# leotimus/binary-recommendation

Hardware: AMD Instinct MI355X
Metric: (user,item) pairs/sec at batch 65536 dim 64 (higher is better)
Workload: dtype f32; 1 GPU; NeuMF-A full training step (trainers/NFC_plain.py graph: 4 embeddings, 128->100->50->10->1, BCE, Keras-Adam adam_dense), embed_dim=64, 1000000 users x 100000 items per GPU, batch 65536 per GPU, uniform ids; global_batch=65536, parallelism=single GPU, steps_per_graph_launch=4, optimizer=adam_dense (deferred replay)

## Files before the change

### binary-recommendation_amd/csrc/adam_math.h

```cpp
#pragma once
#include "common.h"
#include "rows.h"

namespace br {

struct AdamHp {
  float alpha, b1, omb1, b2, omb2, eps;
  const float* alpha_ptr;
};
__device__ __forceinline__ void adam_resolve(AdamHp& h) {
  if (h.alpha_ptr) h.alpha = *h.alpha_ptr;
}

__device__ __forceinline__ float adam_inv_denom(float v, float eps) {
  return __builtin_amdgcn_rcpf(__builtin_amdgcn_sqrtf(v) + eps);
}

__device__ __forceinline__ void adam_update1(float& th, float& m, float& v, float g, const AdamHp& h) {
  m = __builtin_fmaf(h.omb1, g, h.b1 * m);
  v = __builtin_fmaf(h.omb2, g * g, h.b2 * v);
  th = __builtin_fmaf(-(h.alpha * m), adam_inv_denom(v, h.eps), th);
}
__device__ __forceinline__ void adam_update(float4& th, float4& m, float4& v, float4 g, const AdamHp& h) {
  adam_update1(th.x, m.x, v.x, g.x, h); adam_update1(th.y, m.y, v.y, g.y, h);
  adam_update1(th.z, m.z, v.z, g.z, h); adam_update1(th.w, m.w, v.w, g.w, h);
}
__device__ __forceinline__ void adam_update(float2& th, float2& m, float2& v, float2 g, const AdamHp& h) {
  adam_update1(th.x, m.x, v.x, g.x, h); adam_update1(th.y, m.y, v.y, g.y, h);
}
__device__ __forceinline__ void adam_update(float& th, float& m, float& v, float g, const AdamHp& h) {
  adam_update1(th, m, v, g, h);
}

typedef float pk2 __attribute__((ext_vector_type(2)));
__device__ __forceinline__ void adam_decay_pk(pk2& th, pk2& m, pk2& v, float alpha, const AdamHp& h) {
  m = m * h.b1;
  v = v * h.b2;
  pk2 d = {__builtin_amdgcn_sqrtf(v.x), __builtin_amdgcn_sqrtf(v.y)};
  d = d + h.eps;
  const pk2 r = {__builtin_amdgcn_rcpf(d.x), __builtin_amdgcn_rcpf(d.y)};
  th = __builtin_elementwise_fma(-(m * alpha), r, th);
}
__device__ __forceinline__ void adam_decay(float& th, float& m, float& v, float alpha, const AdamHp& h) {
  m = m * h.b1;
  v = v * h.b2;
  th = __builtin_fmaf(-(m * alpha), adam_inv_denom(v, h.eps), th);
}
__device__ __forceinline__ void adam_decay(float2& th, float2& m, float2& v, float alpha, const AdamHp& h) {
  pk2 t = {th.x, th.y}, mm = {m.x, m.y}, vv = {v.x, v.y};
  adam_decay_pk(t, mm, vv, alpha, h);
  th = make_float2(t.x, t.y); m = make_float2(mm.x, mm.y); v = make_float2(vv.x, vv.y);
}
__device__ __forceinline__ void adam_decay(float4& th, float4& m, float4& v, float alpha, const AdamHp& h) {
  pk2 t0 = {th.x, th.y}, m0 = {m.x, m.y}, v0 = {v.x, v.y}, t1 = {th.z, th.w}, m1 = {m.z, m.w}, v1 = {v.z, v.w};
  adam_decay_pk(t0, m0, v0, alpha, h);
  adam_decay_pk(t1, m1, v1, alpha, h);
  th = make_float4(t0.x, t0.y, t1.x, t1.y); m = make_float4(m0.x, m0.y, m1.x, m1.y); v = make_float4(v0.x, v0.y, v1.x, v1.y);
}

__device__ __forceinline__ bool all_zero(float4 a) { return a.x == 0.f && a.y == 0.f && a.z == 0.f && a.w == 0.f; }
__device__ __forceinline__ bool all_zero(float2 a) { return a.x == 0.f && a.y == 0.f; }
__device__ __forceinline__ bool all_zero(float a) { return a == 0.f; }

struct CatchUp {
  const float* m;
  const float* v;
  const int32_t* last;
  const StepStateDev* ss;
  float b1, b2, eps;
};

template <typename V>
__device__ __forceinline__ void adam_replay(V& th, V& m, V& v, uint32_t from, uint32_t upto, const float* ring, const AdamHp& h) {
  if (all_zero(m) && all_zero(v)) return;
  for (uint32_t j = from + 1; j <= upto; ++j) adam_decay(th, m, v, ring[j & (BR_ALPHA_RING - 1)], h);
}

template <typename V>
__device__ __forceinline__ void adam_replay_uniform(V& th, V& m, V& v, uint32_t from, uint32_t upto, const StepStateDev* __restrict__ ss,
                                                    const AdamHp& h) {
  if (__builtin_amdgcn_ballot_w64(!(all_zero(m) && all_zero(v))) == 0) return;
  float a = ss->alpha_hist[(from + 1) & (BR_ALPHA_RING - 1)];
  for (uint32_t j = from + 1; j <= upto; ++j) {
    const float an = ss->alpha_hist[(j + 1) & (BR_ALPHA_RING - 1)];
    adam_decay(th, m, v, a, h);
    a = an;
  }
}

struct FastRp {
  float c, eps_c;
  uint32_t trunc;
};
__device__ __forceinline__ FastRp fast_rp(const StepStateDev* __restrict__ ss) { return FastRp{ss->sqrt_b2, ss->eps_c, ss->trunc}; }

__device__ __forceinline__ void fast_open(pk2 v, float eps, pk2& d, pk2& r) {
  d = (pk2){__builtin_amdgcn_sqrtf(v.x), __builtin_amdgcn_sqrtf(v.y)} + eps;
  r = (pk2){__builtin_amdgcn_rcpf(d.x), __builtin_amdgcn_rcpf(d.y)};
}
__device__ __forceinline__ void fast_open(float v, float eps, float& d, float& r) {
  d = __builtin_amdgcn_sqrtf(v) + eps;
  r = __builtin_amdgcn_rcpf(d);
}
__device__ __forceinline__ void fast_step(pk2& th, pk2& m, pk2& d, pk2& r, float alpha, float b1, const FastRp& f) {
  m = m * b1;
  d = __builtin_elementwise_fma(d, (pk2){f.c, f.c}, (pk2){f.eps_c, f.eps_c});
  r = r * __builtin_elementwise_fma(-d, r, (pk2){2.f, 2.f});
  th = __builtin_elementwise_fma(-(m * alpha), r, th);
}
__device__ __forceinline__ void fast_step(float& th, float& m, float& d, float& r, float alpha, float b1, const FastRp& f) {
  m = m * b1;
  d = __builtin_fmaf(d, f.c, f.eps_c);
  r = r * __builtin_fmaf(-d, r, 2.f);
  th = __builtin_fmaf(-(m * alpha), r, th);
}
template <typename V> struct FastSt;
template <> struct FastSt<float> {
  float th, m, d, r;
  __device__ __forceinline__ void open(float t, float mm, float v, float eps) { th = t; m = mm; fast_open(v, eps, d, r); }
  __device__ __forceinline__ void step(float a, float b1, const FastRp& f) { fast_step(th, m, d, r, a, b1, f); }
  __device__ __forceinline__ float theta() const { return th; }
};
template <> struct FastSt<float2> {
  pk2 th, m, d, r;
  __device__ __forceinline__ void open(float2 t, float2 mm, float2 v, float eps) { th = (pk2){t.x, t.y}; m = (pk2){mm.x, mm.y}; fast_open((pk2){v.x, v.y}, eps, d, r); }
  __device__ __forceinline__ void step(float a, float b1, const FastRp& f) { fast_step(th, m, d, r, a, b1, f); }
  __device__ __forceinline__ float2 theta() const { return make_float2(th.x, th.y); }
};
template <> struct FastSt<float4> {
  pk2 th0, m0, d0, r0, th1, m1, d1, r1;
  __device__ __forceinline__ void open(float4 t, float4 mm, float4 v, float eps) {
    th0 = (pk2){t.x, t.y}; m0 = (pk2){mm.x, mm.y}; fast_open((pk2){v.x, v.y}, eps, d0, r0);
    th1 = (pk2){t.z, t.w}; m1 = (pk2){mm.z, mm.w}; fast_open((pk2){v.z, v.w}, eps, d1, r1);
  }
  __device__ __forceinline__ void step(float a, float b1, const FastRp& f) { fast_step(th0, m0, d0, r0, a, b1, f); fast_step(th1, m1, d1, r1, a, b1, f); }
  __device__ __forceinline__ float4 theta() const { return make_float4(th0.x, th0.y, th1.x, th1.y); }
};
__device__ __forceinline__ uint32_t pow_index(uint32_t k) { return k < (uint32_t)BR_ALPHA_RING ? k : (uint32_t)BR_ALPHA_RING - 1u; }

template <typename V>
__device__ __forceinline__ void fast_moments(V& m, V& v, uint32_t lag, const StepStateDev* __restrict__ ss) {
  const uint32_t k = pow_index(lag);
  m = vmul(m, ss->pow1[k]);
  v = vmul(v, ss->pow2[k]);
}

template <typename V>
__device__ __forceinline__ void adam_replay_fast_uniform(V& th, const V& m, const V& v, uint32_t from, uint32_t upto, const StepStateDev* __restrict__ ss,
                                                         const AdamHp& h) {
  if (__builtin_amdgcn_ballot_w64(!(all_zero(m) && all_zero(v))) == 0) return;
  const FastRp f = fast_rp(ss);
  const uint32_t lag = upto - from;
  const uint32_t end = from + (lag < f.trunc ? lag : f.trunc);
  FastSt<V> st;
  st.open(th, m, v, h.eps);
  uint32_t j = from + 1;
  for (; j + 7 <= end; j += 8) {
    const float* __restrict__ rp = ss->alpha_hist + (j & (BR_ALPHA_RING - 1));
    float a8[8];
#pragma unroll
    for (int k = 0; k < 8; ++k) a8[k] = rp[k];
#pragma unroll
    for (int k = 0; k < 8; ++k) st.step(a8[k], h.b1, f);
  }
  for (; j <= end; ++j) st.step(ss->alpha_hist[j & (BR_ALPHA_RING - 1)], h.b1, f);
  th = st.theta();
}
template <typename V>
__device__ __forceinline__ void adam_replay_fast(V& th, const V& m, const V& v, uint32_t from, uint32_t upto, const float* ring, const FastRp& f,
                                                 const AdamHp& h) {
  if (all_zero(m) && all_zero(v)) return;
  const uint32_t lag = upto - from;
  const uint32_t end = from + (lag < f.trunc ? lag : f.trunc);
  FastSt<V> st;
  st.open(th, m, v, h.eps);
  for (uint32_t j = from + 1; j <= end; ++j) st.step(ring[j & (BR_ALPHA_RING - 1)], h.b1, f);
  th = st.theta();
}

template <bool MOMENTS, typename V>
__device__ __forceinline__ void adam_catch_up_uniform(V& th, V& m, V& v, uint32_t from, uint32_t upto, const StepStateDev* __restrict__ ss, const AdamHp& h) {
  if (ss->fast) {
    adam_replay_fast_uniform(th, m, v, from, upto, ss, h);
    if (MOMENTS) fast_moments(m, v, upto - from, ss);
  } else {
    adam_replay_uniform(th, m, v, from, upto, ss, h);
  }
}
template <bool MOMENTS, typename V>
__device__ __forceinline__ void adam_catch_up(V& th, V& m, V& v, uint32_t from, uint32_t upto, const float* ring, const StepStateDev* __restrict__ ss,
                                              const AdamHp& h) {
  if (ss->fast) {
    adam_replay_fast(th, m, v, from, upto, ring, fast_rp(ss), h);
    if (MOMENTS) fast_moments(m, v, upto - from, ss);
  } else {
    adam_replay(th, m, v, from, upto, ring, h);
  }
}

__device__ __forceinline__ void stage_alpha_ring(float* lds_ring, const StepStateDev* ss) {
  for (int k = threadIdx.x; k < BR_ALPHA_RING; k += blockDim.x) lds_ring[k] = ss->alpha_hist[k];
  __syncthreads();
}

static inline AdamHp make_hp(double alpha, double b1, double b2, double eps) {
  AdamHp h;
  h.alpha = (float)alpha;
  h.b1 = (float)b1;
  h.omb1 = (float)(1.0 - b1);
  h.b2 = (float)b2;
  h.omb2 = (float)(1.0 - b2);
  h.eps = (float)eps;
  const StepStateDev* ss = current_step_state();
  h.alpha_ptr = ss ? &ss->alpha_t : nullptr;
  return h;
}

}
```

### binary-recommendation_amd/csrc/gather.hip

```cpp
#include "common.h"
#include "rows.h"
#include "adam_math.h"
#include "lookup_wave.h"

namespace br {

struct GatherArgs {
  const float* tables[4];
  const void* ids[4];
  float* outs[4];
  int64_t rows[4];
};

template <typename IdT, int VEC, int NT>
__global__ __launch_bounds__(256) void gather_rows_kernel(GatherArgs a, int dim, int chunks,
                                                           int lpr_log2, int64_t batch, int* err) {
  using V = typename VecT<VEC>::type;
  const int lpr = 1 << lpr_log2;
  const int64_t tid = (int64_t)blockIdx.x * blockDim.x + threadIdx.x;
  const int64_t b = tid >> lpr_log2;
  const int lir = (int)(tid & (lpr - 1));
  if (b >= batch) return;
  int64_t id[NT];
  bool ok[NT];
#pragma unroll
  for (int t = 0; t < NT; ++t) {
    id[t] = load_id(reinterpret_cast<const IdT*>(a.ids[t]), b);
    ok[t] = (uint64_t)id[t] < (uint64_t)a.rows[t];
    if (!ok[t] && err && lir == 0) *err = 1;
  }
  for (int c = lir; c < chunks; c += lpr) {
    V v[NT];
#pragma unroll
    for (int t = 0; t < NT; ++t)
      v[t] = ok[t] ? vload<VEC>(a.tables[t] + id[t] * dim + c * VEC) : vzero<VEC>();
#pragma unroll
    for (int t = 0; t < NT; ++t) vstore<VEC>(a.outs[t] + b * dim + c * VEC, v[t]);
  }
}

struct GatherSegJob { const float* table; int64_t rows; const void* ids; float* out; int64_t seg_off; };
struct GatherSegJobs { GatherSegJob j[2]; };
template <typename IdT, int VEC>
__global__ __launch_bounds__(256) void gather_rows_seg_kernel(GatherSegJobs jobs, int dim, int chunks, int lpr_log2, int64_t n, int64_t seg_len, int64_t seg_stride,
                                                               int64_t ld_out, int* err) {
  const GatherSegJob& jb = jobs.j[blockIdx.y];
  const int lpr = 1 << lpr_log2;
  const int64_t tid = (int64_t)blockIdx.x * blockDim.x + threadIdx.x;
  const int64_t b = tid >> lpr_log2;
  const int lir = (int)(tid & (lpr - 1));
  if (b >= n) return;
  const int64_t p = seg_phys(b, seg_len, seg_stride, jb.seg_off);
  const int64_t id = load_id((const IdT*)jb.ids, p);
  const bool ok = (uint64_t)id < (uint64_t)jb.rows;
  if (!ok && err && lir == 0) *err = 1;
  for (int c = lir; c < chunks; c += lpr)
    vstore<VEC>(jb.out + p * ld_out + c * VEC, ok ? vload<VEC>(jb.table + id * dim + c * VEC) : vzero<VEC>());
}

template <int VEC>
__global__ __launch_bounds__(256) void row_dot_kernel(const float* __restrict__ A, const float* __restrict__ Bm,
                                                       float* __restrict__ out, int dim, int chunks,
                                                       int lpr_log2, int64_t batch) {
  const int lpr = 1 << lpr_log2;
  const int64_t tid = (int64_t)blockIdx.x * blockDim.x + threadIdx.x;
  int64_t b = tid >> lpr_log2;
  const int lir = (int)(tid & (lpr - 1));
  const bool live = b < batch;
  if (!live) b = batch - 1;
  float s = 0.f;
  for (int c = lir; c < chunks; c += lpr)
    s += vdot(vload<VEC>(A + b * dim + c * VEC), vload<VEC>(Bm + b * dim + c * VEC));
  s = rowgroup_sum(s, lpr);
  if (live && lir == 0) out[b] = s;
}

template <int VEC>
__global__ __launch_bounds__(256) void row_dot_bwd_kernel(const float* __restrict__ A, const float* __restrict__ Bm,
                                                           const float* __restrict__ dout, float* __restrict__ dA,
                                                           float* __restrict__ dB, int dim, int chunks,
                                                           int lpr_log2, int64_t batch) {
  const int lpr = 1 << lpr_log2;
  const int64_t tid = (int64_t)blockIdx.x * blockDim.x + threadIdx.x;
  const int64_t b = tid >> lpr_log2;
  const int lir = (int)(tid & (lpr - 1));
  if (b >= batch) return;
  const float g = dout[b];
  for (int c = lir; c < chunks; c += lpr) {
    auto va = vload<VEC>(A + b * dim + c * VEC);
    auto vb = vload<VEC>(Bm + b * dim + c * VEC);
    vstore<VEC>(dA + b * dim + c * VEC, vmul(vb, g));
    vstore<VEC>(dB + b * dim + c * VEC, vmul(va, g));
  }
}

template <typename IdT, int VEC>
__global__ __launch_bounds__(256) void neumf_embed_fwd_kernel(
    const float* __restrict__ user_mlp, const float* __restrict__ item_mlp,
    const float* __restrict__ user_mf, const float* __restrict__ item_mf, int64_t ldu, int64_t ldi,
    int64_t user_rows, int64_t item_rows, const IdT* __restrict__ users, const IdT* __restrict__ items,
    int dim, int chunks, int lpr_log2, int64_t batch, int item_first, float* __restrict__ x0,
    float* __restrict__ dot, int* err, float* __restrict__ stash_user, float* __restrict__ stash_item, int64_t ld_stash) {
  using V = typename VecT<VEC>::type;
  const int lpr = 1 << lpr_log2;
  const int64_t tid = (int64_t)blockIdx.x * blockDim.x + threadIdx.x;
  int64_t b = tid >> lpr_log2;
  const int lir = (int)(tid & (lpr - 1));
  const bool live = b < batch;
  if (!live) b = batch - 1;
  const int64_t u = load_id(users, b), i = load_id(items, b);
  const bool uok = (uint64_t)u < (uint64_t)user_rows, iok = (uint64_t)i < (uint64_t)item_rows;
  if ((!uok || !iok) && err && lir == 0) *err = 1;
  float* xrow = x0 + b * (2 * (int64_t)dim);
  const int uoff = item_first ? dim : 0, ioff = item_first ? 0 : dim;
  float s = 0.f;
  for (int c = lir; c < chunks; c += lpr) {
    V um = uok ? vload<VEC>(user_mlp + u * ldu + c * VEC) : vzero<VEC>();
    V im = iok ? vload<VEC>(item_mlp + i * ldi + c * VEC) : vzero<VEC>();
    V uf = uok ? vload<VEC>(user_mf + u * ldu + c * VEC) : vzero<VEC>();
    V vf = iok ? vload<VEC>(item_mf + i * ldi + c * VEC) : vzero<VEC>();
    if (live) {
      vstore<VEC>(xrow + uoff + c * VEC, um);
      vstore<VEC>(xrow + ioff + c * VEC, im);
      if (stash_user) {
        vstore<VEC>(stash_user + b * ld_stash + c * VEC, uf);
        vstore<VEC>(stash_item + b * ld_stash + c * VEC, vf);
      }
    }
    s += vdot(uf, vf);
  }
  s = rowgroup_sum(s, lpr);
  if (live && lir == 0) dot[b] = s;
}

template <typename IdT, int VEC>
__global__ __launch_bounds__(256) void neumf_embed_fwd_deferred_kernel(
    const float* __restrict__ user_tab, const float* __restrict__ user_m, const float* __restrict__ user_v,
    const int32_t* __restrict__ user_last, const float* __restrict__ item_tab, const float* __restrict__ item_m,
    const float* __restrict__ item_v, const int32_t* __restrict__ item_last, int64_t user_rows, int64_t item_rows,
    const IdT* __restrict__ users, const IdT* __restrict__ items, int dim, int chunks, int lpr_log2, int64_t batch,
    int item_first, const StepStateDev* __restrict__ ss, AdamHp h, float* __restrict__ x0, float* __restrict__ dot,
    float* __restrict__ stash_user, float* __restrict__ stash_item, int64_t ld_stash, int* err) {
  using V = typename VecT<VEC>::type;
  __shared__ float ring[BR_ALPHA_RING];
  stage_alpha_ring(ring, ss);
  const int lpr = 1 << lpr_log2;
  const int64_t tid = (int64_t)blockIdx.x * blockDim.x + threadIdx.x;
  int64_t b = tid >> lpr_log2;
  const int lir = (int)(tid & (lpr - 1));
  const bool live = b < batch;
  if (!live) b = batch - 1;
  int64_t u = load_id(users, b), i = load_id(items, b);
  const bool uok = (uint64_t)u < (uint64_t)user_rows, iok = (uint64_t)i < (uint64_t)item_rows;
  if ((!uok || !iok) && err && lir == 0) *err = 1;
  if (!uok) u = 0;
  if (!iok) i = 0;
  const uint32_t t = ss->step;
  const uint32_t lu = (uint32_t)user_last[u], li = (uint32_t)item_last[i];
  const int64_t ld = 2 * (int64_t)dim;
  float* xrow = x0 + b * ld;
  const int uoff = item_first ? dim : 0, ioff = item_first ? 0 : dim;
  float s = 0.f;
  for (int c = lir; c < chunks; c += lpr) {
    const int64_t uo = u * ld + c * VEC, io = i * ld + c * VEC;
    V um = vload<VEC>(user_tab + uo), uf = vload<VEC>(user_tab + uo + dim);
    V im = vload<VEC>(item_tab + io), vf = vload<VEC>(item_tab + io + dim);
    if (lu + 1 < t) {
      V m0 = vload<VEC>(user_m + uo), v0 = vload<VEC>(user_v + uo), m1 = vload<VEC>(user_m + uo + dim), v1 = vload<VEC>(user_v + uo + dim);
      adam_catch_up<false>(um, m0, v0, lu, t - 1, ring, ss, h);
      adam_catch_up<false>(uf, m1, v1, lu, t - 1, ring, ss, h);
    }
    if (li + 1 < t) {
      V m0 = vload<VEC>(item_m + io), v0 = vload<VEC>(item_v + io), m1 = vload<VEC>(item_m + io + dim), v1 = vload<VEC>(item_v + io + dim);
      adam_catch_up<false>(im, m0, v0, li, t - 1, ring, ss, h);
      adam_catch_up<false>(vf, m1, v1, li, t - 1, ring, ss, h);
    }
    if (!uok) { um = vzero<VEC>(); uf = vzero<VEC>(); }
    if (!iok) { im = vzero<VEC>(); vf = vzero<VEC>(); }
    if (live) {
      vstore<VEC>(xrow + uoff + c * VEC, um);
      vstore<VEC>(xrow + ioff + c * VEC, im);
      vstore<VEC>(stash_user + b * ld_stash + c * VEC, uf);
      vstore<VEC>(stash_item + b * ld_stash + c * VEC, vf);
    }
    s += vdot(uf, vf);
  }
  s = rowgroup_sum(s, lpr);
  if (live && lir == 0) dot[b] = s;
}

template <typename IdT, int VEC>
__global__ __launch_bounds__(256) void neumf_embed_fwd_deferred_wave_kernel(const LookupArgs a) {
  const int64_t b = (int64_t)blockIdx.x * 4 + __builtin_amdgcn_readfirstlane((int)(threadIdx.x >> 6));
  if (b >= a.batch) return;
  lookup_wave_pair<IdT, VEC>(a, b, (int)(threadIdx.x & 63));
}

template <typename IdT, int VEC>
__global__ __launch_bounds__(256) void gather_rows_deferred_kernel(
    const float* __restrict__ table, const float* __restrict__ M, const float* __restrict__ Vv, const int32_t* __restrict__ last,
    int64_t rows, int dim, int chunks, int lpr_log2, const IdT* __restrict__ ids, int64_t n, const StepStateDev* __restrict__ ss,
    AdamHp h, float* __restrict__ out, int64_t ld_out, int* err) {
  using V = typename VecT<VEC>::type;
  __shared__ float ring[BR_ALPHA_RING];
  stage_alpha_ring(ring, ss);
  const int lpr = 1 << lpr_log2;
  const int64_t tid = (int64_t)blockIdx.x * blockDim.x + threadIdx.x;
  const int64_t b = tid >> lpr_log2;
  const int lir = (int)(tid & (lpr - 1));
  if (b >= n) return;
  int64_t r = load_id(ids, b);
  const bool ok = (uint64_t)r < (uint64_t)rows;
  if (!ok) { if (err && lir == 0) *err = 1; r = 0; }
  const uint32_t t = ss->step, seen = (uint32_t)last[r];
  for (int c = lir; c < chunks; c += lpr) {
    const int64_t off = r * dim + c * VEC;
    V th = vload<VEC>(table + off);
    if (seen + 1 < t) {
      V m = vload<VEC>(M + off), v = vload<VEC>(Vv + off);
      adam_catch_up<false>(th, m, v, seen, t - 1, ring, ss, h);
    }
    vstore<VEC>(out + b * ld_out + c * VEC, ok ? th : vzero<VEC>());
  }
}

template <typename IdT, int VEC>
__global__ __launch_bounds__(256) void gather_rows_deferred_wave_kernel(
    const float* __restrict__ table, const float* __restrict__ M, const float* __restrict__ Vv, const int32_t* __restrict__ last,
    int64_t rows, const IdT* __restrict__ ids, int64_t n, const StepStateDev* __restrict__ ss, AdamHp h, float* __restrict__ out,
    int64_t ld_out, int* err) {
  using V = typename VecT<VEC>::type;
  constexpr int dim = 64 * VEC;
  const int64_t b = (int64_t)blockIdx.x * 4 + __builtin_amdgcn_readfirstlane((int)(threadIdx.x >> 6));
  if (b >= n) return;
  const int lane = (int)(threadIdx.x & 63);
  int64_t r = load_id(ids, b);
  const bool ok = (uint64_t)r < (uint64_t)rows;
  if (!ok) { if (err && lane == 0) *err = 1; r = 0; }
  const uint32_t t = ss->step, seen = (uint32_t)last[r];
  const int64_t off = r * dim + lane * VEC;
  V th = vload<VEC>(table + off);
  if (seen + 1 < t) {
    V m = vload<VEC>(M + off), v = vload<VEC>(Vv + off);
    adam_catch_up_uniform<false>(th, m, v, seen, t - 1, ss, h);
  }
  vstore<VEC>(out + b * ld_out + lane * VEC, ok ? th : vzero<VEC>());
}

template <typename IdT, int VEC>
__global__ __launch_bounds__(256) void gather_rows_deferred_wave_pair_kernel(GatherDefJobs jobs, const StepStateDev* __restrict__ ss, AdamHp h,
                                                                              int64_t ld_out, int* err) {
  const GatherDefJob& jb = jobs.j[blockIdx.y];
  const int64_t b = (int64_t)blockIdx.x * 4 + __builtin_amdgcn_readfirstlane((int)(threadIdx.x >> 6));
  if (b >= jb.n) return;
  gather_deferred_wave_row<IdT, VEC>(jobs, jb, b, (int)(threadIdx.x & 63), ss, h, ld_out, err);
}

template <int VEC>
__global__ __launch_bounds__(256) void mf_grad_inplace_kernel(float* su, float* si, int64_t ld, const float* __restrict__ ddot,
                                                               int64_t batch, int chunks) {
  using V = typename VecT<VEC>::type;
  const int64_t e = (int64_t)blockIdx.x * blockDim.x + threadIdx.x;
  if (e >= batch * chunks) return;
  const int64_t b = e / chunks;
  const int c = (int)(e - b * chunks);
  const float g = ddot[b];
  const V u = vload<VEC>(su + b * ld + c * VEC), i = vload<VEC>(si + b * ld + c * VEC);
  vstore<VEC>(su + b * ld + c * VEC, vmul(i, g));
  vstore<VEC>(si + b * ld + c * VEC, vmul(u, g));
}

template <typename IdT, int VEC>
__global__ __launch_bounds__(256) void neumf_embed_bwd_kernel(
    const float* __restrict__ user_mf, const float* __restrict__ item_mf, int64_t ldu, int64_t ldi,
    int64_t user_rows, int64_t item_rows, const IdT* __restrict__ users, const IdT* __restrict__ items,
    int dim, int chunks, int lpr_log2, int64_t batch, int item_first, const float* __restrict__ dx0,
    const float* __restrict__ ddot, float* __restrict__ g_user_mlp, float* __restrict__ g_item_mlp,
    float* __restrict__ g_user_mf, float* __restrict__ g_item_mf, int64_t ldg, int out_by_id) {
  using V = typename VecT<VEC>::type;
  const int lpr = 1 << lpr_log2;
  const int64_t tid = (int64_t)blockIdx.x * blockDim.x + threadIdx.x;
  const int64_t b = tid >> lpr_log2;
  const int lir = (int)(tid & (lpr - 1));
  if (b >= batch) return;
  const int64_t u = load_id(users, b), i = load_id(items, b);
  const bool uok = (uint64_t)u < (uint64_t)user_rows, iok = (uint64_t)i < (uint64_t)item_rows;
  const int64_t ou = out_by_id ? (uok ? u : -1) : b, oi = out_by_id ? (iok ? i : -1) : b;
  const float g = ddot[b];
  const int uoff = item_first ? dim : 0, ioff = item_first ? 0 : dim;
  for (int c = lir; c < chunks; c += lpr) {
    V uf = uok ? vload<VEC>(user_mf + u * ldu + c * VEC) : vzero<VEC>();
    V vf = iok ? vload<VEC>(item_mf + i * ldi + c * VEC) : vzero<VEC>();
    if (ou >= 0) vstore<VEC>(g_user_mf + ou * ldg + c * VEC, vmul(vf, g));
    if (oi >= 0) vstore<VEC>(g_item_mf + oi * ldg + c * VEC, vmul(uf, g));
    if (g_user_mlp) {
      const float* xr = dx0 + b * (2 * (int64_t)dim);
      if (ou >= 0) vstore<VEC>(g_user_mlp + ou * ldg + c * VEC, vload<VEC>(xr + uoff + c * VEC));
      if (oi >= 0) vstore<VEC>(g_item_mlp + oi * ldg + c * VEC, vload<VEC>(xr + ioff + c * VEC));
    }
  }
}

template <typename IdT, int VEC>
__global__ __launch_bounds__(256) void bpr_fwd_bwd_kernel(
    const float* __restrict__ user_table, const float* __restrict__ item_table, int64_t user_rows,
    int64_t item_rows, const IdT* __restrict__ users, const IdT* __restrict__ pos,
    const IdT* __restrict__ neg, int dim, int chunks, int lpr_log2, int64_t batch, float inv_batch,
    float* __restrict__ per_triplet, double* __restrict__ loss_sum, float* __restrict__ g_user,
    float* __restrict__ g_item, int* err) {
  using V = typename VecT<VEC>::type;
  const int lpr = 1 << lpr_log2;
  const int64_t tid = (int64_t)blockIdx.x * blockDim.x + threadIdx.x;
  int64_t b = tid >> lpr_log2;
  const int lir = (int)(tid & (lpr - 1));
  const bool live = b < batch;
  if (!live) b = batch - 1;
  const int64_t u = load_id(users, b), p = load_id(pos, b), n = load_id(neg, b);
  const bool uok = (uint64_t)u < (uint64_t)user_rows;
  const bool pok = (uint64_t)p < (uint64_t)item_rows, nok = (uint64_t)n < (uint64_t)item_rows;
  if (!(uok && pok && nok) && err && lir == 0) *err = 1;
  float sp = 0.f, sn = 0.f;
  const bool one_pass = chunks <= lpr;
  V eu = vzero<VEC>(), ep = vzero<VEC>(), en = vzero<VEC>();
  if (one_pass) {
    if (lir < chunks) {
      eu = uok ? vload<VEC>(user_table + u * dim + lir * VEC) : vzero<VEC>();
      ep = pok ? vload<VEC>(item_table + p * dim + lir * VEC) : vzero<VEC>();
      en = nok ? vload<VEC>(item_table + n * dim + lir * VEC) : vzero<VEC>();
    }
    sp = vdot(eu, ep);
    sn = vdot(eu, en);
  } else {
    for (int c = lir; c < chunks; c += lpr) {
      V a = uok ? vload<VEC>(user_table + u * dim + c * VEC) : vzero<VEC>();
      V bp = pok ? vload<VEC>(item_table + p * dim + c * VEC) : vzero<VEC>();
      V bn = nok ? vload<VEC>(item_table + n * dim + c * VEC) : vzero<VEC>();
      sp += vdot(a, bp);
      sn += vdot(a, bn);
    }
  }
  sp = rowgroup_sum(sp, lpr);
  sn = rowgroup_sum(sn, lpr);
  const float x = sp - sn;
  const float s = sigmoidf_acc(x);
  const float l = 1.f - s;
  const float dx = -s * (1.f - s) * inv_batch;
  if (live) {
    if (per_triplet && lir == 0) per_triplet[b] = l;
    float* gu = g_user + b * dim;
    float* gp = g_item + b * dim;
    float* gn = g_item + (batch + b) * dim;
    if (one_pass) {
      if (lir < chunks) {
        vstore<VEC>(gu + lir * VEC, vmul(vsub(ep, en), dx));
        vstore<VEC>(gp + lir * VEC, vmul(eu, dx));
        vstore<VEC>(gn + lir * VEC, vmul(eu, -dx));
      }
    } else {
      for (int c = lir; c < chunks; c += lpr) {
        V a = uok ? vload<VEC>(user_table + u * dim + c * VEC) : vzero<VEC>();
        V bp = pok ? vload<VEC>(item_table + p * dim + c * VEC) : vzero<VEC>();
        V bn = nok ? vload<VEC>(item_table + n * dim + c * VEC) : vzero<VEC>();
        vstore<VEC>(gu + c * VEC, vmul(vsub(bp, bn), dx));
        vstore<VEC>(gp + c * VEC, vmul(a, dx));
        vstore<VEC>(gn + c * VEC, vmul(a, -dx));
      }
    }
  }
  __shared__ double red[4];
  double contrib = (live && lir == 0) ? (double)l : 0.0;
  contrib = wave_sum_d(contrib);
  const int wave = threadIdx.x >> 6, lane = threadIdx.x & 63;
  if (lane == 0) red[wave] = contrib;
  __syncthreads();
  if (threadIdx.x == 0 && loss_sum) atomicAdd(loss_sum + (blockIdx.x & (BR_SUM_SLOTS - 1)), red[0] + red[1] + red[2] + red[3]);
}

}

using namespace br;

static inline unsigned grid_for_rows(int64_t batch, int lpr_log2) {
  const int64_t rows_per_block = 256 >> lpr_log2;
  return (unsigned)ceil_div(batch, rows_per_block);
}

extern "C" int brGatherRows(int n_tables, const float* const* tables, const int64_t* table_rows,
                            const void* const* ids, float* const* outs, int dim, int64_t batch,
                            int id_type, int* err_flag, brStream stream) {
  BR_CHECK_ARG(n_tables >= 1 && n_tables <= BR_MAX_TABLES, "brGatherRows: n_tables %d out of [1,%d]", n_tables, BR_MAX_TABLES);
  BR_CHECK_ARG(dim >= 1 && batch >= 0, "brGatherRows: bad dim/batch");
  BR_CHECK_ARG(id_type == BR_IDS_I32 || id_type == BR_IDS_I64, "brGatherRows: bad id_type %d", id_type);
  if (batch == 0) return BR_OK;
  for (int t = 0; t < n_tables; ++t)
    BR_CHECK_ARG(tables[t] && outs[t] && table_rows[t] > 0, "brGatherRows: null table/out %d", t);
  const RowGeom g = row_geom(dim);
  hipStream_t s = (hipStream_t)stream;
  const unsigned grid = grid_for_rows(batch, g.lpr_log2);
  for (int t0 = 0; t0 < n_tables; t0 += 4) {
    const int nt = (n_tables - t0) < 4 ? (n_tables - t0) : 4;
    GatherArgs a{};
    for (int t = 0; t < nt; ++t) {
      a.tables[t] = tables[t0 + t];
      a.ids[t] = ids ? ids[t0 + t] : nullptr;
      a.outs[t] = outs[t0 + t];
      a.rows[t] = table_rows[t0 + t];
    }
#define LAUNCH_G(NT) \
  BR_DISPATCH_ID(id_type, BR_DISPATCH_VEC(g.vec, (gather_rows_kernel<IdT, VEC, NT><<<grid, 256, 0, s>>>(a, dim, g.chunks, g.lpr_log2, batch, err_flag))))
    switch (nt) {
      case 1: LAUNCH_G(1); break;
      case 2: LAUNCH_G(2); break;
      case 3: LAUNCH_G(3); break;
      default: LAUNCH_G(4); break;
    }
#undef LAUNCH_G
    BR_CHECK_LAUNCH("brGatherRows");
  }
  return BR_OK;
}

extern "C" int brRowDot(const float* a, const float* b, float* out, int dim, int64_t batch, brStream stream) {
  BR_CHECK_ARG(a && b && out && dim >= 1 && batch >= 0, "brRowDot: bad args");
  if (batch == 0) return BR_OK;
  const RowGeom g = row_geom(dim);
  BR_DISPATCH_VEC(g.vec, (row_dot_kernel<VEC><<<grid_for_rows(batch, g.lpr_log2), 256, 0, (hipStream_t)stream>>>(
                             a, b, out, dim, g.chunks, g.lpr_log2, batch)));
  BR_CHECK_LAUNCH("brRowDot");
  return BR_OK;
}

extern "C" int brRowDotBackward(const float* a, const float* b, const float* dout, float* da, float* db,
                                int dim, int64_t batch, brStream stream) {
  BR_CHECK_ARG(a && b && dout && da && db && dim >= 1 && batch >= 0, "brRowDotBackward: bad args");
  if (batch == 0) return BR_OK;
  const RowGeom g = row_geom(dim);
  BR_DISPATCH_VEC(g.vec, (row_dot_bwd_kernel<VEC><<<grid_for_rows(batch, g.lpr_log2), 256, 0, (hipStream_t)stream>>>(
                             a, b, dout, da, db, dim, g.chunks, g.lpr_log2, batch)));
  BR_CHECK_LAUNCH("brRowDotBackward");
  return BR_OK;
}

extern "C" int brNeumfEmbedForward(const float* user_mlp, const float* item_mlp, const float* user_mf,
                                   const float* item_mf, int64_t ld_user, int64_t ld_item, int64_t user_rows,
                                   int64_t item_rows, const void* users, const void* items, int id_type, int dim,
                                   int64_t batch, int item_first, float* x0, float* dot, int* err_flag, brStream stream) {
  return brNeumfEmbedForwardStash(user_mlp, item_mlp, user_mf, item_mf, ld_user, ld_item, user_rows, item_rows, users, items, id_type, dim, batch, item_first, x0, dot,
                                  nullptr, nullptr, 0, err_flag, stream);
}

extern "C" int brNeumfEmbedForwardStash(const float* user_mlp, const float* item_mlp, const float* user_mf,
                                        const float* item_mf, int64_t ld_user, int64_t ld_item, int64_t user_rows,
                                        int64_t item_rows, const void* users, const void* items, int id_type, int dim,
                                        int64_t batch, int item_first, float* x0, float* dot, float* stash_user, float* stash_item, int64_t ld_stash,
                                        int* err_flag, brStream stream) {
  BR_CHECK_ARG(user_mlp && item_mlp && user_mf && item_mf && x0 && dot, "brNeumfEmbedForward: null pointer");
  BR_CHECK_ARG((stash_user == nullptr) == (stash_item == nullptr) && (!stash_user || ld_stash >= dim), "brNeumfEmbedForwardStash: both stashes (ld >= dim) or neither");
  BR_CHECK_ARG(dim >= 1 && batch >= 0 && user_rows > 0 && item_rows > 0, "brNeumfEmbedForward: bad sizes");
  BR_CHECK_ARG(ld_user >= dim && ld_item >= dim, "brNeumfEmbedForward: row strides < dim");
  BR_CHECK_ARG(id_type == BR_IDS_I32 || id_type == BR_IDS_I64, "brNeumfEmbedForward: bad id_type");
  if (batch == 0) return BR_OK;
  const RowGeom g = row_geom_ld(dim, vec_width({ld_user, ld_item, stash_user ? ld_stash : 0}, {stash_user, stash_item}));
  const unsigned grid = grid_for_rows(batch, g.lpr_log2);
  hipStream_t s = (hipStream_t)stream;
  BR_DISPATCH_ID(id_type, BR_DISPATCH_VEC(g.vec, (neumf_embed_fwd_kernel<IdT, VEC><<<grid, 256, 0, s>>>(
                                                     user_mlp, item_mlp, user_mf, item_mf, ld_user, ld_item, user_rows, item_rows, (const IdT*)users, (const IdT*)items, dim,
                                                     g.chunks, g.lpr_log2, batch, item_first, x0, dot, err_flag, stash_user, stash_item, ld_stash))));
  BR_CHECK_LAUNCH("brNeumfEmbedForward");
  return BR_OK;
}

extern "C" int brNeumfEmbedForwardDeferred(const float* user_tab, const float* user_m, const float* user_v, const int32_t* user_last,
                                           const float* item_tab, const float* item_m, const float* item_v, const int32_t* item_last,
                                           int64_t user_rows, int64_t item_rows, const void* users, const void* items, int id_type,
                                           int dim, int64_t batch, int item_first, const void* step_state, double beta1, double beta2,
                                           double eps, float* x0, float* dot, float* stash_user, float* stash_item, int64_t ld_stash,
                                           int* err_flag, brStream stream) {
  BR_CHECK_ARG(user_tab && user_m && user_v && user_last && item_tab && item_m && item_v && item_last && step_state && x0 && dot &&
                   stash_user && stash_item, "brNeumfEmbedForwardDeferred: null pointer");
  BR_CHECK_ARG(dim >= 1 && batch >= 0 && user_rows > 0 && item_rows > 0 && ld_stash >= dim, "brNeumfEmbedForwardDeferred: bad sizes");
  BR_CHECK_ARG(id_type == BR_IDS_I32 || id_type == BR_IDS_I64, "brNeumfEmbedForwardDeferred: bad id_type");
  if (batch == 0) return BR_OK;
  const RowGeom g = row_geom_ld(dim, vec_width({ld_stash}));
  const unsigned grid = grid_for_rows(batch, g.lpr_log2);
  const AdamHp h = make_hp(0.0, beta1, beta2, eps);
  const StepStateDev* ss = (const StepStateDev*)step_state;
  hipStream_t s = (hipStream_t)stream;
  const int wvec = wave_pair_vec(dim);
  if (wave_rows_enabled() && wvec && ld_stash % wvec == 0 &&
      ((reinterpret_cast<uintptr_t>(stash_user) | reinterpret_cast<uintptr_t>(stash_item) | reinterpret_cast<uintptr_t>(x0)) & (4 * wvec - 1)) == 0) {
    const unsigned wgrid = (unsigned)ceil_div(batch, 4);
    const LookupArgs la{user_tab, user_m, user_v, user_last, item_tab, item_m, item_v, item_last, user_rows, item_rows, users, items, batch, item_first, ss, h,
                        x0, dot, stash_user, stash_item, ld_stash, err_flag};
    BR_DISPATCH_ID(id_type, { if (wvec == 2) neumf_embed_fwd_deferred_wave_kernel<IdT, 2><<<wgrid, 256, 0, s>>>(la); else neumf_embed_fwd_deferred_wave_kernel<IdT, 4><<<wgrid, 256, 0, s>>>(la); });
    BR_CHECK_LAUNCH("brNeumfEmbedForwardDeferred(wave)");
    return BR_OK;
  }
  BR_DISPATCH_ID(id_type, BR_DISPATCH_VEC(g.vec, (neumf_embed_fwd_deferred_kernel<IdT, VEC><<<grid, 256, 0, s>>>(
                                                     user_tab, user_m, user_v, user_last, item_tab, item_m, item_v, item_last, user_rows, item_rows, (const IdT*)users,
                                                     (const IdT*)items, dim, g.chunks, g.lpr_log2, batch, item_first, ss, h, x0, dot, stash_user, stash_item, ld_stash, err_flag))));
  BR_CHECK_LAUNCH("brNeumfEmbedForwardDeferred");
  return BR_OK;
}

extern "C" int brGatherRowsDeferred(const float* table, const float* m, const float* v, const int32_t* last, int64_t table_rows, int dim,
                                    const void* ids, int id_type, int64_t n, const void* step_state, double beta1, double beta2,
                                    double eps, float* out, int64_t ld_out, int* err_flag, brStream stream) {
  BR_CHECK_ARG(table && m && v && last && step_state && out && dim >= 1 && table_rows > 0 && n >= 0 && ld_out >= dim, "brGatherRowsDeferred: bad args");
  BR_CHECK_ARG(id_type == BR_IDS_I32 || id_type == BR_IDS_I64, "brGatherRowsDeferred: bad id_type");
  if (n == 0) return BR_OK;
  BR_CHECK_ARG(ids != nullptr, "brGatherRowsDeferred: null ids");
  const RowGeom g = row_geom_ld(dim, ld_out);
  const unsigned grid = grid_for_rows(n, g.lpr_log2);
  const AdamHp h = make_hp(0.0, beta1, beta2, eps);
  const StepStateDev* ss = (const StepStateDev*)step_state;
  hipStream_t s = (hipStream_t)stream;
  const int wvec = wave_row_vec(dim);
  if (wave_rows_enabled() && wvec && ld_out % wvec == 0 && (reinterpret_cast<uintptr_t>(out) & (4 * wvec - 1)) == 0) {
    const unsigned wgrid = (unsigned)ceil_div(n, 4);
    BR_DISPATCH_ID(id_type, BR_DISPATCH_VEC(wvec, (gather_rows_deferred_wave_kernel<IdT, VEC><<<wgrid, 256, 0, s>>>(table, m, v, last, table_rows, (const IdT*)ids, n, ss, h, out,
                                                                                                                 ld_out, err_flag))));
    BR_CHECK_LAUNCH("brGatherRowsDeferred(wave)");
    return BR_OK;
  }
  BR_DISPATCH_ID(id_type, BR_DISPATCH_VEC(g.vec, (gather_rows_deferred_kernel<IdT, VEC><<<grid, 256, 0, s>>>(table, m, v, last, table_rows, dim, g.chunks, g.lpr_log2, (const IdT*)ids, n,
                                                                                                          ss, h, out, ld_out, err_flag))));
  BR_CHECK_LAUNCH("brGatherRowsDeferred");
  return BR_OK;
}

extern "C" int brGatherRowsDeferredPair(const float* table_a, const float* m_a, const float* v_a, const int32_t* last_a, int64_t rows_a, const void* ids_a,
                                        float* out_a, const float* table_b, const float* m_b, const float* v_b, const int32_t* last_b, int64_t rows_b,
                                        const void* ids_b, float* out_b, int dim, int id_type, int64_t n, int64_t n_b, const void* step_state, double beta1,
                                        double beta2, double eps, int64_t ld_out, int* err_flag, brStream stream) {
  if (n_b == 0) n_b = n;
  BR_CHECK_ARG(table_a && m_a && v_a && last_a && ids_a && out_a && table_b && m_b && v_b && last_b && ids_b && out_b && step_state && rows_a > 0 && rows_b > 0 &&
                   n >= 0 && n_b >= 0 && ld_out >= dim, "brGatherRowsDeferredPair: bad args");
  BR_CHECK_ARG(id_type == BR_IDS_I32 || id_type == BR_IDS_I64, "brGatherRowsDeferredPair: bad id_type");
  if (n == 0 && n_b == 0) return BR_OK;
  const int wvec = wave_row_vec(dim);
  const bool wave_ok = wvec && ld_out % wvec == 0 && ((reinterpret_cast<uintptr_t>(out_a) | reinterpret_cast<uintptr_t>(out_b)) & (4 * wvec - 1)) == 0;
  if (!wave_ok) {
    const int rc = brGatherRowsDeferred(table_a, m_a, v_a, last_a, rows_a, dim, ids_a, id_type, n, step_state, beta1, beta2, eps, out_a, ld_out, err_flag, stream);
    if (rc != BR_OK) return rc;
    return brGatherRowsDeferred(table_b, m_b, v_b, last_b, rows_b, dim, ids_b, id_type, n_b, step_state, beta1, beta2, eps, out_b, ld_out, err_flag, stream);
  }
  GatherDefJobs J;
  J.j[0] = GatherDefJob{table_a, m_a, v_a, last_a, rows_a, ids_a, out_a, n};
  J.j[1] = GatherDefJob{table_b, m_b, v_b, last_b, rows_b, ids_b, out_b, n_b};
  const AdamHp h = make_hp(0.0, beta1, beta2, eps);
  const StepStateDev* ss = (const StepStateDev*)step_state;
  const dim3 grid((unsigned)ceil_div(n > n_b ? n : n_b, 4), 2);
  hipStream_t s = (hipStream_t)stream;
  BR_DISPATCH_ID(id_type, BR_DISPATCH_VEC(wvec, (gather_rows_deferred_wave_pair_kernel<IdT, VEC><<<grid, 256, 0, s>>>(J, ss, h, ld_out, err_flag))));
  BR_CHECK_LAUNCH("brGatherRowsDeferredPair");
  return BR_OK;
}

extern "C" int brGatherRowsDeferredPairSeg(const float* table_a, const float* m_a, const float* v_a, const int32_t* last_a, int64_t rows_a, const float* table_b,
                                           const float* m_b, const float* v_b, const int32_t* last_b, int64_t rows_b, const void* ids, float* out, int dim,
                                           int id_type, int64_t n, int64_t seg_len, int64_t seg_stride, int64_t seg_off_a, int64_t seg_off_b,
                                           const void* step_state, double beta1, double beta2, double eps, int64_t ld_out, int* err_flag, brStream stream) {
  BR_CHECK_ARG(table_a && m_a && v_a && last_a && table_b && m_b && v_b && last_b && ids && out && step_state && rows_a > 0 && rows_b > 0 && n >= 0 && ld_out >= dim,
               "brGatherRowsDeferredPairSeg: bad args");
  BR_CHECK_ARG(id_type == BR_IDS_I32 || id_type == BR_IDS_I64, "brGatherRowsDeferredPairSeg: bad id_type");
  BR_CHECK_ARG(seg_len >= 1 && seg_stride >= seg_len && seg_off_a >= 0 && seg_off_b >= 0, "brGatherRowsDeferredPairSeg: bad segment geometry");
  if (n == 0) return BR_OK;
  const int wvec = wave_row_vec(dim);
  BR_CHECK_ARG(wvec && ld_out % wvec == 0 && (reinterpret_cast<uintptr_t>(out) & (4 * wvec - 1)) == 0,
               "brGatherRowsDeferredPairSeg: rows of 64 / 128 / 256 floats (one wave per row)");
  GatherDefJobs J;
  J.j[0] = GatherDefJob{table_a, m_a, v_a, last_a, rows_a, ids, out, n, seg_off_a};
  J.j[1] = GatherDefJob{table_b, m_b, v_b, last_b, rows_b, ids, out, n, seg_off_b};
  J.seg_len = seg_len; J.seg_stride = seg_stride;
  const AdamHp h = make_hp(0.0, beta1, beta2, eps);
  const StepStateDev* ss = (const StepStateDev*)step_state;
  const dim3 grid((unsigned)ceil_div(n, 4), 2);
  hipStream_t s = (hipStream_t)stream;
  BR_DISPATCH_ID(id_type, BR_DISPATCH_VEC(wvec, (gather_rows_deferred_wave_pair_kernel<IdT, VEC><<<grid, 256, 0, s>>>(J, ss, h, ld_out, err_flag))));
  BR_CHECK_LAUNCH("brGatherRowsDeferredPairSeg");
  return BR_OK;
}

extern "C" int brGatherRowsPairSeg(const float* table_a, int64_t rows_a, const float* table_b, int64_t rows_b, const void* ids, float* out, int dim, int id_type,
                                   int64_t n, int64_t seg_len, int64_t seg_stride, int64_t seg_off_a, int64_t seg_off_b, int64_t ld_out, int* err_flag,
                                   brStream stream) {
  BR_CHECK_ARG(table_a && table_b && ids && out && rows_a > 0 && rows_b > 0 && n >= 0 && dim >= 1 && ld_out >= dim, "brGatherRowsPairSeg: bad args");
  BR_CHECK_ARG(id_type == BR_IDS_I32 || id_type == BR_IDS_I64, "brGatherRowsPairSeg: bad id_type");
  BR_CHECK_ARG(seg_len >= 1 && seg_stride >= seg_len && seg_off_a >= 0 && seg_off_b >= 0, "brGatherRowsPairSeg: bad segment geometry");
  if (n == 0) return BR_OK;
  const RowGeom g = row_geom_ld(dim, vec_width({ld_out}, {out}));
  GatherSegJobs J;
  J.j[0] = GatherSegJob{table_a, rows_a, ids, out, seg_off_a};
  J.j[1] = GatherSegJob{table_b, rows_b, ids, out, seg_off_b};
  const dim3 grid(grid_for_rows(n, g.lpr_log2), 2);
  hipStream_t s = (hipStream_t)stream;
  BR_DISPATCH_ID(id_type, BR_DISPATCH_VEC(g.vec, (gather_rows_seg_kernel<IdT, VEC><<<grid, 256, 0, s>>>(J, dim, g.chunks, g.lpr_log2, n, seg_len, seg_stride, ld_out, err_flag))));
  BR_CHECK_LAUNCH("brGatherRowsPairSeg");
  return BR_OK;
}

extern "C" int brMfGradInplace(float* stash_user, float* stash_item, int64_t ld, const float* ddot, int64_t batch, int dim, brStream stream) {
  BR_CHECK_ARG(stash_user && stash_item && ddot && dim >= 1 && ld >= dim && batch >= 0, "brMfGradInplace: bad args");
  if (batch == 0) return BR_OK;
  const RowGeom g = row_geom_ld(dim, vec_width({ld}));
  const unsigned grid = (unsigned)ceil_div(batch * g.chunks, 256);
  BR_DISPATCH_VEC(g.vec, (mf_grad_inplace_kernel<VEC><<<grid, 256, 0, (hipStream_t)stream>>>(stash_user, stash_item, ld, ddot, batch, g.chunks)));
  BR_CHECK_LAUNCH("brMfGradInplace");
  return BR_OK;
}

extern "C" int brNeumfEmbedBackward(const float* user_mf, const float* item_mf, int64_t ld_user, int64_t ld_item,
                                    int64_t user_rows, int64_t item_rows, const void* users, const void* items,
                                    int id_type, int dim, int64_t batch, int item_first, const float* dx0,
                                    const float* ddot, float* g_user_mlp, float* g_item_mlp, float* g_user_mf,
                                    float* g_item_mf, int64_t ldg, int out_rows_by_id, brStream stream) {
  BR_CHECK_ARG(user_mf && item_mf && ddot && g_user_mf && g_item_mf, "brNeumfEmbedBackward: null pointer");
  BR_CHECK_ARG((g_user_mlp == nullptr) == (g_item_mlp == nullptr), "brNeumfEmbedBackward: g_*_mlp both or neither");
  BR_CHECK_ARG(!g_user_mlp || dx0, "brNeumfEmbedBackward: dx0 required for g_*_mlp");
  BR_CHECK_ARG(ld_user >= dim && ld_item >= dim && ldg >= dim, "brNeumfEmbedBackward: row strides < dim");
  BR_CHECK_ARG(id_type == BR_IDS_I32 || id_type == BR_IDS_I64, "brNeumfEmbedBackward: bad id_type");
  if (batch == 0) return BR_OK;
  const RowGeom g = row_geom_ld(dim, vec_width({ld_user, ld_item, ldg}));
  const unsigned grid = grid_for_rows(batch, g.lpr_log2);
  hipStream_t s = (hipStream_t)stream;
  BR_DISPATCH_ID(id_type, BR_DISPATCH_VEC(g.vec, (neumf_embed_bwd_kernel<IdT, VEC><<<grid, 256, 0, s>>>(
                                                     user_mf, item_mf, ld_user, ld_item, user_rows, item_rows, (const IdT*)users, (const IdT*)items, dim, g.chunks, g.lpr_log2,
                                                     batch, item_first, dx0, ddot, g_user_mlp, g_item_mlp, g_user_mf, g_item_mf, ldg, out_rows_by_id))));
  BR_CHECK_LAUNCH("brNeumfEmbedBackward");
  return BR_OK;
}

extern "C" int brBprForwardBackward(const float* user_table, const float* item_table, int64_t user_rows,
                                    int64_t item_rows, const void* users, const void* pos, const void* neg,
                                    int id_type, int dim, int64_t batch, float inv_batch, float* per_triplet,
                                    double* loss_sum, float* g_user, float* g_item, int* err_flag, brStream stream) {
  BR_CHECK_ARG(user_table && item_table && users && pos && neg && g_user && g_item, "brBprForwardBackward: null pointer");
  BR_CHECK_ARG(dim >= 1 && batch >= 0 && user_rows > 0 && item_rows > 0, "brBprForwardBackward: bad sizes");
  BR_CHECK_ARG(id_type == BR_IDS_I32 || id_type == BR_IDS_I64, "brBprForwardBackward: bad id_type");
  if (batch == 0) return BR_OK;
  const RowGeom g = row_geom(dim);
  const unsigned grid = grid_for_rows(batch, g.lpr_log2);
  hipStream_t s = (hipStream_t)stream;
  BR_DISPATCH_ID(id_type, BR_DISPATCH_VEC(g.vec, (bpr_fwd_bwd_kernel<IdT, VEC><<<grid, 256, 0, s>>>(user_table, item_table, user_rows, item_rows, (const IdT*)users, (const IdT*)pos,
                                                                                                 (const IdT*)neg, dim, g.chunks, g.lpr_log2, batch, inv_batch, per_triplet, loss_sum,
                                                                                                 g_user, g_item, err_flag))));
  BR_CHECK_LAUNCH("brBprForwardBackward");
  return BR_OK;
}
```

### binary-recommendation_amd/csrc/lookup_wave.h

```cpp
#pragma once
#include "common.h"
#include "rows.h"
#include "adam_math.h"
#include <stdlib.h>

namespace br {

struct LookupArgs {
  const float *user_tab, *user_m, *user_v; const int32_t* user_last;
  const float *item_tab, *item_m, *item_v; const int32_t* item_last;
  int64_t user_rows, item_rows;
  const void *users, *items;
  int64_t batch; int item_first;
  const StepStateDev* ss; AdamHp h;
  float *x0, *dot, *stash_user, *stash_item; int64_t ld_stash; int* err;
  uint32_t step_add = 0;
  uint32_t spec = 0;
};
static inline uint32_t lookup_spec(int64_t, int64_t, int64_t) {
  static const int forced = [] { const char* e = getenv("BR_LOOKUP_SPEC"); return e ? atoi(e) : 0; }();
  return (uint32_t)forced & 3u;
}

template <typename IdT, int VEC>
__device__ __forceinline__ void lookup_wave_pair(const LookupArgs& a, int64_t b, int lane) {
  using V = typename VecT<VEC>::type;
  constexpr int dim = 32 * VEC;
  constexpr int64_t ld = 2 * dim;
  const float* __restrict__ user_tab = a.user_tab; const float* __restrict__ item_tab = a.item_tab;
  const StepStateDev* __restrict__ ss = a.ss;
  const int col = lane * VEC;
  int64_t u = load_id((const IdT*)a.users, b), i = load_id((const IdT*)a.items, b);
  const bool uok = (uint64_t)u < (uint64_t)a.user_rows, iok = (uint64_t)i < (uint64_t)a.item_rows;
  if ((!uok || !iok) && a.err && lane == 0) *a.err = 1;
  if (!uok) u = 0;
  if (!iok) i = 0;
  const uint32_t t = ss->step + a.step_add;
  const uint32_t lu = (uint32_t)a.user_last[u], li = (uint32_t)a.item_last[i];
  const int64_t uo = u * ld + col, io = i * ld + col;
  V ur = vload<VEC>(user_tab + uo), ir = vload<VEC>(item_tab + io);
  V um = vzero<VEC>(), uv = vzero<VEC>(), im = vzero<VEC>(), iv = vzero<VEC>();
  if ((a.spec & 1u) || lu + 1 < t) { um = vload<VEC>(a.user_m + uo); uv = vload<VEC>(a.user_v + uo); }
  if ((a.spec & 2u) || li + 1 < t) { im = vload<VEC>(a.item_m + io); iv = vload<VEC>(a.item_v + io); }
  if (li + 1 < t) adam_catch_up_uniform<false>(ir, im, iv, li, t - 1, ss, a.h);
  if (lu + 1 < t) adam_catch_up_uniform<false>(ur, um, uv, lu, t - 1, ss, a.h);
  if (!uok) ur = vzero<VEC>();
  if (!iok) ir = vzero<VEC>();
  const bool mlp = lane < 32;
  const int uoff = a.item_first ? dim : 0, ioff = a.item_first ? 0 : dim;
  vstore<VEC>(mlp ? a.x0 + b * ld + uoff + col : a.stash_user + b * a.ld_stash + (col - dim), ur);
  vstore<VEC>(mlp ? a.x0 + b * ld + ioff + col : a.stash_item + b * a.ld_stash + (col - dim), ir);
  float s;
  if constexpr (VEC == 4) {
    s = 0.f + vdot(ur, ir);
    s += __shfl_xor(s, 16, 64);
  } else {
    static_assert(VEC == 2, "wave lookup: embed_dim 64 or 128");
    const float e = __builtin_fmaf(ur.y, ir.y, ur.x * ir.x);
    const float prev = __shfl_up(e, 1, 64);
    s = 0.f + __builtin_fmaf(ur.y, ir.y, __builtin_fmaf(ur.x, ir.x, prev));
    s += __shfl_xor(s, 16, 64);
  }
  s += __shfl_xor(s, 8, 64);
  s += __shfl_xor(s, 4, 64);
  s += __shfl_xor(s, 2, 64);
  if constexpr (VEC == 4) s += __shfl_xor(s, 1, 64);
  if (lane == 63) a.dot[b] = s;
}

template <typename IdT>
__device__ __forceinline__ void lookup_half_pair(const LookupArgs& a, int64_t b, int lane) {
  constexpr int dim = 64;
  constexpr int64_t ld = 2 * dim;
  const StepStateDev* __restrict__ ss = a.ss;
  const bool it = lane >= 32;
  const int col = (lane & 31) * 4;
  int64_t u = load_id((const IdT*)a.users, b), i = load_id((const IdT*)a.items, b);
  const bool uok = (uint64_t)u < (uint64_t)a.user_rows, iok = (uint64_t)i < (uint64_t)a.item_rows;
  if ((!uok || !iok) && a.err && lane == 0) *a.err = 1;
  if (!uok) u = 0;
  if (!iok) i = 0;
  const uint32_t t = ss->step + a.step_add;
  const uint32_t lu = (uint32_t)a.user_last[u], li = (uint32_t)a.item_last[i];
  const FastRp f = fast_rp(ss);
  uint32_t lag_u = lu + 1 < t ? t - 1 - lu : 0u, lag_i = li + 1 < t ? t - 1 - li : 0u;
  const int64_t off = (it ? i : u) * ld + col;
  const float4 th = vload<4>((it ? a.item_tab : a.user_tab) + off);
  float4 m = vzero<4>(), v = vzero<4>();
  if (it ? lag_i > 0 : lag_u > 0) { m = vload<4>((it ? a.item_m : a.user_m) + off); v = vload<4>((it ? a.item_v : a.user_v) + off); }
  float4 out = th;
  lag_u = lag_u < f.trunc ? lag_u : f.trunc; lag_i = lag_i < f.trunc ? lag_i : f.trunc;
  const uint32_t steps = lag_u > lag_i ? lag_u : lag_i, mine = it ? lag_i : lag_u;
  if (steps > 0 && __builtin_amdgcn_ballot_w64(!(all_zero(m) && all_zero(v))) != 0) {
    FastSt<float4> st;
    st.open(th, m, v, a.h.eps);
    uint32_t k = 1;
    for (; k + 7 <= steps; k += 8) {
      const float* __restrict__ ru = ss->alpha_hist + ((lu + k) & (BR_ALPHA_RING - 1));
      const float* __restrict__ ri = ss->alpha_hist + ((li + k) & (BR_ALPHA_RING - 1));
      float au[8], ai[8];
#pragma unroll
      for (int q = 0; q < 8; ++q) { au[q] = ru[q]; ai[q] = ri[q]; }
#pragma unroll
      for (int q = 0; q < 8; ++q) st.step(k + q <= mine ? (it ? ai[q] : au[q]) : 0.f, a.h.b1, f);
    }
    for (; k <= steps; ++k) {
      const float au = ss->alpha_hist[(lu + k) & (BR_ALPHA_RING - 1)], ai = ss->alpha_hist[(li + k) & (BR_ALPHA_RING - 1)];
      st.step(k <= mine ? (it ? ai : au) : 0.f, a.h.b1, f);
    }
    out = st.theta();
  }
  if (it ? !iok : !uok) out = vzero<4>();
  const bool mlp = col < dim;
  const int uoff = a.item_first ? dim : 0, ioff = a.item_first ? 0 : dim;
  float* dst = mlp ? a.x0 + b * ld + (it ? ioff : uoff) + col : (it ? a.stash_item : a.stash_user) + b * a.ld_stash + (col - dim);
  vstore<4>(dst, out);
  float4 other;
  other.x = __shfl_xor(out.x, 32, 64); other.y = __shfl_xor(out.y, 32, 64); other.z = __shfl_xor(out.z, 32, 64); other.w = __shfl_xor(out.w, 32, 64);
  float sdot = 0.f + (it ? vdot(other, out) : vdot(out, other));
  sdot += __shfl_xor(sdot, 8, 64);
  sdot += __shfl_xor(sdot, 4, 64);
  sdot += __shfl_xor(sdot, 2, 64);
  sdot += __shfl_xor(sdot, 1, 64);
  if (lane == 63) a.dot[b] = sdot;
}

template <typename IdT, int VEC, int R>
__device__ __forceinline__ void lookup_wave_pairs(const LookupArgs& a, int64_t b0, int lane) {
  using V = typename VecT<VEC>::type;
  constexpr int dim = 32 * VEC;
  constexpr int64_t ld = 2 * dim;
  const float* __restrict__ user_tab = a.user_tab; const float* __restrict__ item_tab = a.item_tab;
  const StepStateDev* __restrict__ ss = a.ss;
  const int col = lane * VEC;
  const uint32_t t = ss->step + a.step_add;
  int64_t u[R], i[R], bq[R];
  bool live[R], uok[R], iok[R];
#pragma unroll
  for (int q = 0; q < R; ++q) {
    live[q] = b0 + q < a.batch;
    bq[q] = live[q] ? b0 + q : a.batch - 1;
    u[q] = load_id((const IdT*)a.users, bq[q]); i[q] = load_id((const IdT*)a.items, bq[q]);
  }
  uint32_t lu[R], li[R];
#pragma unroll
  for (int q = 0; q < R; ++q) {
    uok[q] = (uint64_t)u[q] < (uint64_t)a.user_rows; iok[q] = (uint64_t)i[q] < (uint64_t)a.item_rows;
    if ((!uok[q] || !iok[q]) && a.err && lane == 0 && live[q]) *a.err = 1;
    if (!uok[q]) u[q] = 0;
    if (!iok[q]) i[q] = 0;
    lu[q] = (uint32_t)a.user_last[u[q]]; li[q] = (uint32_t)a.item_last[i[q]];
  }
  V ur[R], ir[R], um[R], uv[R], im[R], iv[R];
#pragma unroll
  for (int q = 0; q < R; ++q) {
    const int64_t uo = u[q] * ld + col, io = i[q] * ld + col;
    ur[q] = vload<VEC>(user_tab + uo); ir[q] = vload<VEC>(item_tab + io);
    um[q] = vzero<VEC>(); uv[q] = vzero<VEC>(); im[q] = vzero<VEC>(); iv[q] = vzero<VEC>();
    if (lu[q] + 1 < t) { um[q] = vload<VEC>(a.user_m + uo); uv[q] = vload<VEC>(a.user_v + uo); }
    if (li[q] + 1 < t) { im[q] = vload<VEC>(a.item_m + io); iv[q] = vload<VEC>(a.item_v + io); }
  }
  const bool mlp = lane < 32;
  const int uoff = a.item_first ? dim : 0, ioff = a.item_first ? 0 : dim;
#pragma unroll
  for (int q = 0; q < R; ++q) {
    if (li[q] + 1 < t) adam_catch_up_uniform<false>(ir[q], im[q], iv[q], li[q], t - 1, ss, a.h);
    if (lu[q] + 1 < t) adam_catch_up_uniform<false>(ur[q], um[q], uv[q], lu[q], t - 1, ss, a.h);
    if (!uok[q]) ur[q] = vzero<VEC>();
    if (!iok[q]) ir[q] = vzero<VEC>();
    if (!live[q]) continue;
    const int64_t b = bq[q];
    vstore<VEC>(mlp ? a.x0 + b * ld + uoff + col : a.stash_user + b * a.ld_stash + (col - dim), ur[q]);
    vstore<VEC>(mlp ? a.x0 + b * ld + ioff + col : a.stash_item + b * a.ld_stash + (col - dim), ir[q]);
    float s;
    if constexpr (VEC == 4) {
      s = 0.f + vdot(ur[q], ir[q]);
      s += __shfl_xor(s, 16, 64);
    } else {
      static_assert(VEC == 2 || VEC == 4, "wave lookup: embed_dim 64 or 128");
      const float e = __builtin_fmaf(ur[q].y, ir[q].y, ur[q].x * ir[q].x);
      const float prev = __shfl_up(e, 1, 64);
      s = 0.f + __builtin_fmaf(ur[q].y, ir[q].y, __builtin_fmaf(ur[q].x, ir[q].x, prev));
      s += __shfl_xor(s, 16, 64);
    }
    s += __shfl_xor(s, 8, 64);
    s += __shfl_xor(s, 4, 64);
    s += __shfl_xor(s, 2, 64);
    if constexpr (VEC == 4) s += __shfl_xor(s, 1, 64);
    if (lane == 63) a.dot[b] = s;
  }
}

struct GatherDefJob { const float* table; const float* M; const float* Vv; const int32_t* last; int64_t rows; const void* ids; float* out; int64_t n; int64_t seg_off = 0; };
struct GatherDefJobs {
  GatherDefJob j[2];
  int64_t seg_len = 0, seg_stride = 0;
  uint32_t step_add = 0;
};
template <typename IdT, int VEC>
__device__ __forceinline__ void gather_deferred_wave_row(const GatherDefJobs& jobs, const GatherDefJob& jb, int64_t b, int lane, const StepStateDev* __restrict__ ss,
                                                         const AdamHp& h, int64_t ld_out, int* err) {
  using V = typename VecT<VEC>::type;
  constexpr int dim = 64 * VEC;
  b = seg_phys(b, jobs.seg_len, jobs.seg_stride, jb.seg_off);
  int64_t r = load_id((const IdT*)jb.ids, b);
  const bool ok = (uint64_t)r < (uint64_t)jb.rows;
  if (!ok) { if (err && lane == 0) *err = 1; r = 0; }
  const uint32_t t = ss->step + jobs.step_add, seen = (uint32_t)jb.last[r];
  const int64_t off = r * dim + lane * VEC;
  V th = vload<VEC>(jb.table + off);
  if (seen + 1 < t) {
    V m = vload<VEC>(jb.M + off), v = vload<VEC>(jb.Vv + off);
    adam_catch_up_uniform<false>(th, m, v, seen, t - 1, ss, h);
  }
  vstore<VEC>(jb.out + b * ld_out + lane * VEC, ok ? th : vzero<VEC>());
}

template <typename IdT, int VEC, int R>
__device__ __forceinline__ void gather_deferred_wave_rows(const GatherDefJobs& jobs, int64_t b0, int lane, const StepStateDev* __restrict__ ss, const AdamHp& h,
                                                          int64_t ld_out, int* err) {
  using V = typename VecT<VEC>::type;
  constexpr int dim = 64 * VEC;
  const int64_t n_a = jobs.j[0].n, n_all = n_a + jobs.j[1].n;
  const uint32_t t = ss->step + jobs.step_add;
  int which[R];
  int64_t pos[R], row[R];
  bool live[R], ok[R];
#pragma unroll
  for (int q = 0; q < R; ++q) {
    const int64_t b = b0 + q;
    live[q] = b < n_all;
    const int64_t bc = live[q] ? b : n_all - 1;
    which[q] = bc < n_a ? 0 : 1;
    const GatherDefJob& jb = jobs.j[which[q]];
    pos[q] = seg_phys(which[q] ? bc - n_a : bc, jobs.seg_len, jobs.seg_stride, jb.seg_off);
    row[q] = load_id((const IdT*)jb.ids, pos[q]);
  }
  uint32_t seen[R];
#pragma unroll
  for (int q = 0; q < R; ++q) {
    const GatherDefJob& jb = jobs.j[which[q]];
    ok[q] = (uint64_t)row[q] < (uint64_t)jb.rows;
    if (!ok[q]) { if (err && lane == 0 && live[q]) *err = 1; row[q] = 0; }
    seen[q] = (uint32_t)jb.last[row[q]];
  }
  V th[R], m[R], v[R];
#pragma unroll
  for (int q = 0; q < R; ++q) {
    const GatherDefJob& jb = jobs.j[which[q]];
    const int64_t off = row[q] * dim + lane * VEC;
    th[q] = vload<VEC>(jb.table + off);
    m[q] = vzero<VEC>(); v[q] = vzero<VEC>();
    if (seen[q] + 1 < t) { m[q] = vload<VEC>(jb.M + off); v[q] = vload<VEC>(jb.Vv + off); }
  }
#pragma unroll
  for (int q = 0; q < R; ++q) {
    if (seen[q] + 1 < t) adam_catch_up_uniform<false>(th[q], m[q], v[q], seen[q], t - 1, ss, h);
    if (live[q]) vstore<VEC>(jobs.j[which[q]].out + pos[q] * ld_out + lane * VEC, ok[q] ? th[q] : vzero<VEC>());
  }
}

template <typename IdT>
__device__ __forceinline__ void gather_deferred_group4(const GatherDefJobs& jobs, int64_t b0, int lane, const StepStateDev* __restrict__ ss, const AdamHp& h,
                                                       int64_t ld_out, int* err) {
  constexpr int dim = 64;
  const int64_t n_a = jobs.j[0].n, n_all = n_a + jobs.j[1].n;
  const uint32_t t = ss->step + jobs.step_add;
  const int q = lane >> 4, col = (lane & 15) * 4;
  const int64_t b = b0 + q;
  const bool live = b < n_all;
  const int64_t bc = live ? b : n_all - 1;
  const int which = bc < n_a ? 0 : 1;
  const GatherDefJob& ja = jobs.j[0];
  const GatherDefJob& jb = jobs.j[1];
  const int64_t pos = seg_phys(which ? bc - n_a : bc, jobs.seg_len, jobs.seg_stride, which ? jb.seg_off : ja.seg_off);
  int64_t row = which ? load_id((const IdT*)jb.ids, pos) : load_id((const IdT*)ja.ids, pos);
  const int64_t rows = which ? jb.rows : ja.rows;
  const bool ok = (uint64_t)row < (uint64_t)rows;
  if (!ok) { if (err && live && (lane & 15) == 0) *err = 1; row = 0; }
  const uint32_t seen = (uint32_t)(which ? jb.last : ja.last)[row];
  const FastRp f = fast_rp(ss);
  uint32_t lag = seen + 1 < t ? t - 1 - seen : 0u;
  const int64_t off = row * dim + col;
  float4 th = vload<4>((which ? jb.table : ja.table) + off);
  float4 m = vzero<4>(), v = vzero<4>();
  if (lag > 0) { m = vload<4>((which ? jb.M : ja.M) + off); v = vload<4>((which ? jb.Vv : ja.Vv) + off); }
  lag = lag < f.trunc ? lag : f.trunc;
  uint32_t steps = lag;
  steps = max(steps, (uint32_t)__shfl_xor((int)steps, 16, 64));
  steps = max(steps, (uint32_t)__shfl_xor((int)steps, 32, 64));
  steps = (uint32_t)__builtin_amdgcn_readfirstlane((int)steps);
  if (steps > 0 && __builtin_amdgcn_ballot_w64(!(all_zero(m) && all_zero(v))) != 0) {
    const uint32_t s0 = (uint32_t)__builtin_amdgcn_readlane((int)seen, 0), s1 = (uint32_t)__builtin_amdgcn_readlane((int)seen, 16);
    const uint32_t s2 = (uint32_t)__builtin_amdgcn_readlane((int)seen, 32), s3 = (uint32_t)__builtin_amdgcn_readlane((int)seen, 48);
    FastSt<float4> st;
    st.open(th, m, v, h.eps);
    uint32_t k = 1;
    for (; k + 7 <= steps; k += 8) {
      const float* __restrict__ r0 = ss->alpha_hist + ((s0 + k) & (BR_ALPHA_RING - 1));
      const float* __restrict__ r1 = ss->alpha_hist + ((s1 + k) & (BR_ALPHA_RING - 1));
      const float* __restrict__ r2 = ss->alpha_hist + ((s2 + k) & (BR_ALPHA_RING - 1));
      const float* __restrict__ r3 = ss->alpha_hist + ((s3 + k) & (BR_ALPHA_RING - 1));
      float a0[8], a1[8], a2[8], a3[8];
#pragma unroll
      for (int e = 0; e < 8; ++e) { a0[e] = r0[e]; a1[e] = r1[e]; a2[e] = r2[e]; a3[e] = r3[e]; }
#pragma unroll
      for (int e = 0; e < 8; ++e) {
        const float al = q == 0 ? a0[e] : (q == 1 ? a1[e] : (q == 2 ? a2[e] : a3[e]));
        st.step(k + e <= lag ? al : 0.f, h.b1, f);
      }
    }
    for (; k <= steps; ++k) {
      const float a0 = ss->alpha_hist[(s0 + k) & (BR_ALPHA_RING - 1)], a1 = ss->alpha_hist[(s1 + k) & (BR_ALPHA_RING - 1)];
      const float a2 = ss->alpha_hist[(s2 + k) & (BR_ALPHA_RING - 1)], a3 = ss->alpha_hist[(s3 + k) & (BR_ALPHA_RING - 1)];
      const float al = q == 0 ? a0 : (q == 1 ? a1 : (q == 2 ? a2 : a3));
      st.step(k <= lag ? al : 0.f, h.b1, f);
    }
    th = st.theta();
  }
  if (live) vstore<4>((which ? jb.out : ja.out) + pos * ld_out + col, ok ? th : vzero<4>());
}

}
```

### binary-recommendation_amd/csrc/row_index.hip

```cpp
#include "common.h"
#include "rows.h"
#include "adam_math.h"
#include "lookup_wave.h"
#include "dense.h"
#include "step_state.h"

#include <hipcub/hipcub.hpp>

namespace br {

template <typename IdT>
__global__ void sort_prep_kernel(const IdT* __restrict__ ids, int64_t upper, IdT* __restrict__ keys, int32_t* __restrict__ p, int64_t n) {
  const int64_t i = (int64_t)blockIdx.x * blockDim.x + threadIdx.x;
  if (i < n) {
    p[i] = (int32_t)i;
    const int64_t id = (int64_t)ids[i];
    keys[i] = (upper > 0 && (uint64_t)id >= (uint64_t)upper) ? (IdT)upper : (IdT)id;
  }
}

static inline int bits_for(int64_t upper) {
  int bits = 1;
  while (bits < 63 && ((int64_t)1 << bits) < upper) ++bits;
  return bits;
}

template <typename IdT>
static int64_t sort_temp_bytes(int64_t n) {
  size_t bytes = 0;
  (void)hipcub::DeviceRadixSort::SortPairs((void*)nullptr, bytes, (const IdT*)nullptr, (IdT*)nullptr, (const int32_t*)nullptr,
                                     (int32_t*)nullptr, (int)n, 0, (int)sizeof(IdT) * 8, (hipStream_t)0);
  return (int64_t)bytes;
}

}

using namespace br;

static inline int64_t align256(int64_t x) { return (x + 255) & ~(int64_t)255; }

constexpr int kChunkS = 2048, kThreadsS = 256, kChunkL = 8192, kThreadsL = 1024, kRankMaxChunks = 64;
constexpr int64_t kChunkSwitchN = 16384;
constexpr int64_t kRankMaxN = (int64_t)kChunkL * kRankMaxChunks;
struct IdxJob {
  const void* ids;
  void* sorted_ids;
  int32_t* sorted_pos;
  uint32_t* ck;
  uint32_t* cp;
  uint32_t upper;
  int end_bit;
  int64_t seg_len = 0, seg_stride = 0, seg_off = 0;
  int64_t n = 0;
  int n_chunks = 0;
};

struct IdxJobs { IdxJob j[2]; };

template <typename IdT, int kChunk, int kSortThreads>
__device__ __forceinline__ void chunk_sort_block(const IdxJobs& jobs, int64_t n, int chunk, int which) {
  constexpr int IPT = kChunk / kSortThreads;
  using Sort = hipcub::BlockRadixSort<uint32_t, kSortThreads, IPT, uint32_t>;
  __shared__ typename Sort::TempStorage tmp;
  const IdxJob& job = jobs.j[which];
  if (job.n) n = job.n;
  const IdT* ids = (const IdT*)job.ids;
  const int64_t base = (int64_t)chunk * kChunk + threadIdx.x * IPT;
  uint32_t k[IPT], p[IPT];
#pragma unroll
  for (int q = 0; q < IPT; ++q) {
    const int64_t e = base + q;
    const int64_t pe = seg_phys(e, job.seg_len, job.seg_stride, job.seg_off);
    const int64_t id = e < n ? (int64_t)ids[pe] : -1;
    k[q] = e < n ? (((uint64_t)id < (uint64_t)job.upper) ? (uint32_t)id : job.upper) : job.upper + 1u;
    p[q] = (uint32_t)pe;
  }
  Sort(tmp).Sort(k, p, 0, job.end_bit);
#pragma unroll
  for (int q = 0; q < IPT; ++q)
    if (base + q < n) { job.ck[base + q] = k[q]; job.cp[base + q] = p[q]; }
}
template <typename IdT, int kChunk, int kSortThreads>
__global__ __launch_bounds__(kSortThreads) void chunk_sort_kernel(IdxJobs jobs, int64_t n) {
  chunk_sort_block<IdT, kChunk, kSortThreads>(jobs, n, (int)blockIdx.x, (int)blockIdx.y);
}

template <typename IdT, int VEC, int R>
__global__ __launch_bounds__(kThreadsL, 8) void lookup_sort_kernel(const LookupArgs a, IdxJobs jobs, int64_t n, int n_chunks) {
  const int n_sort = 2 * n_chunks;
  if ((int)blockIdx.x < n_sort) {
    chunk_sort_block<IdT, kChunkL, kThreadsL>(jobs, n, (int)blockIdx.x % n_chunks, (int)blockIdx.x / n_chunks);
    return;
  }
  const int64_t b = (((int64_t)blockIdx.x - n_sort) * (kThreadsL / 64) + __builtin_amdgcn_readfirstlane((int)(threadIdx.x >> 6))) * (R < 1 ? 1 : R);
  if (b >= a.batch) return;
  if constexpr (R == 0) {
    if (a.ss->fast) lookup_half_pair<IdT>(a, b, (int)(threadIdx.x & 63));
    else lookup_wave_pair<IdT, VEC>(a, b, (int)(threadIdx.x & 63));
  } else if constexpr (R == 1) lookup_wave_pair<IdT, VEC>(a, b, (int)(threadIdx.x & 63));
  else lookup_wave_pairs<IdT, VEC, R>(a, b, (int)(threadIdx.x & 63));
}
static int lookup_pairs_per_wave() {
  static const int r = [] { const char* e = getenv("BR_LOOKUP_PAIRS"); const int v = e ? atoi(e) : 1; return (v == 0 || v == 2) ? v : 1; }();
  return r;
}

template <int VEC> constexpr int kGatherRowsPerWave = VEC == 1 ? 4 : (VEC == 2 ? 2 : 1);
template <typename IdT, int VEC>
__global__ __launch_bounds__(kThreadsL) void gather_sort_kernel(const GatherDefJobs gj, const StepStateDev* __restrict__ ss, const AdamHp h, int64_t ld_out, int* err,
                                                                IdxJobs jobs, int n_sort_a, int n_sort_b, bool gather_group4_enabled) {
  const int n_sort = n_sort_a + n_sort_b;
  if ((int)blockIdx.x < n_sort) {
    const int which = (int)blockIdx.x < n_sort_a ? 0 : 1;
    chunk_sort_block<IdT, kChunkL, kThreadsL>(jobs, 0, which ? (int)blockIdx.x - n_sort_a : (int)blockIdx.x, which);
    return;
  }
  constexpr int R = kGatherRowsPerWave<VEC>;
  const int64_t b0 = (((int64_t)blockIdx.x - n_sort) * (kThreadsL / 64) + __builtin_amdgcn_readfirstlane((int)(threadIdx.x >> 6))) * R;
  if (b0 >= gj.j[0].n + gj.j[1].n) return;
  if constexpr (VEC == 1) {
    if (ss->fast && (ld_out & 3) == 0 && gather_group4_enabled) { gather_deferred_group4<IdT>(gj, b0, (int)(threadIdx.x & 63), ss, h, ld_out, err); return; }
  }
  gather_deferred_wave_rows<IdT, VEC, R>(gj, b0, (int)(threadIdx.x & 63), ss, h, ld_out, err);
}

template <typename IdT, int kChunk>
__global__ __launch_bounds__(256) void chunk_rank_kernel(IdxJobs jobs, int64_t n, int n_chunks, const StepAdvance adv) {
  if (adv.st && blockIdx.x == gridDim.x - 1) {
    if (blockIdx.y == 0) step_state_advance_block(adv);
    return;
  }
  const IdxJob& job = jobs.j[blockIdx.y];
  if (job.n) { n = job.n; n_chunks = job.n_chunks; }
  const int64_t e = (int64_t)blockIdx.x * 256 + threadIdx.x;
  if (e >= n) return;
  const int c = (int)(e / kChunk);
  const uint32_t key = job.ck[e];
  uint32_t rank = (uint32_t)(e - (int64_t)c * kChunk);
  constexpr int G = 8;
  for (int c0 = 0; c0 < n_chunks; c0 += G) {
    uint32_t lo[G], len[G];
#pragma unroll
    for (int u = 0; u < G; ++u) {
      const int cc = c0 + u;
      const int64_t left = n - (int64_t)cc * kChunk;
      len[u] = (cc < n_chunks && cc != c) ? (uint32_t)(left < kChunk ? left : kChunk) : 0u;
      lo[u] = 0u;
    }
#pragma unroll
    for (int step = kChunk; step > 0; step >>= 1) {
      uint32_t v[G];
#pragma unroll
      for (int u = 0; u < G; ++u) {
        const uint32_t idx = lo[u] + (uint32_t)step;
        const uint32_t at = idx <= len[u] ? idx - 1u : 0u;
        v[u] = job.ck[(int64_t)(c0 + u < n_chunks ? c0 + u : 0) * kChunk + at];
      }
#pragma unroll
      for (int u = 0; u < G; ++u) {
        const uint32_t idx = lo[u] + (uint32_t)step;
        const uint32_t lt = (c0 + u < c) ? (v[u] <= key ? 1u : 0u) : (v[u] < key ? 1u : 0u);
        lo[u] += (idx <= len[u] ? lt : 0u) * (uint32_t)step;
      }
    }
#pragma unroll
    for (int u = 0; u < G; ++u) rank += lo[u];
  }
  ((IdT*)job.sorted_ids)[rank] = (IdT)key;
  job.sorted_pos[rank] = (int32_t)job.cp[e];
}

static bool rank_path_ok(int64_t n, int64_t upper) { return n <= kRankMaxN && upper > 0 && upper < ((int64_t)1 << 31) - 2; }

static int index_build_rank(IdxJobs& jobs, int n_jobs, int id_type, int64_t n, hipStream_t s) {
  const bool large = n > kChunkSwitchN;
  const int n_chunks = (int)ceil_div(n, large ? kChunkL : kChunkS);
  const dim3 g1((unsigned)n_chunks, (unsigned)n_jobs), g2((unsigned)ceil_div(n, 256), (unsigned)n_jobs);
  BR_DISPATCH_ID(id_type, {
    if (large) { chunk_sort_kernel<IdT, kChunkL, kThreadsL><<<g1, kThreadsL, 0, s>>>(jobs, n); probe_split(BR_TAG_INDEX_SORT, s); chunk_rank_kernel<IdT, kChunkL><<<g2, 256, 0, s>>>(jobs, n, n_chunks, StepAdvance{}); }
    else { chunk_sort_kernel<IdT, kChunkS, kThreadsS><<<g1, kThreadsS, 0, s>>>(jobs, n); probe_split(BR_TAG_INDEX_SORT, s); chunk_rank_kernel<IdT, kChunkS><<<g2, 256, 0, s>>>(jobs, n, n_chunks, StepAdvance{}); }
  });
  BR_CHECK_LAUNCH("brRowIndexBuild");
  return BR_OK;
}
static IdxJob make_job(const void* ids, void* sorted_ids, int32_t* sorted_pos, void* workspace, int64_t n, int64_t upper) {
  IdxJob j{};
  j.ids = ids; j.sorted_ids = sorted_ids; j.sorted_pos = sorted_pos;
  j.ck = (uint32_t*)workspace;
  j.cp = (uint32_t*)((char*)workspace + align256(n * 4));
  j.upper = (uint32_t)upper;
  j.end_bit = bits_for(upper + 2);
  return j;
}

extern "C" int64_t brRowIndexWorkspaceBytes(int64_t n, int id_type) {
  if (n <= 0) return 256;
  const int64_t iota = align256(n * 4);
  const int64_t tmp = id_type == BR_IDS_I64 ? sort_temp_bytes<int64_t>(n) : sort_temp_bytes<int32_t>(n);
  const int64_t rank = 2 * align256(n * 4);
  const int64_t sort = iota + align256(n * 8) + align256(tmp);
  return (sort > rank ? sort : rank) + 256;
}

extern "C" int brRowIndexBuild(const void* ids, int id_type, int64_t n, int64_t id_upper_bound, void* sorted_ids,
                               int32_t* sorted_pos, void* workspace, int64_t workspace_bytes, brStream stream) {
  BR_CHECK_ARG(id_type == BR_IDS_I32 || id_type == BR_IDS_I64, "brRowIndexBuild: bad id_type");
  BR_CHECK_ARG(n >= 0 && n < ((int64_t)1 << 31), "brRowIndexBuild: n out of range");
  if (n == 0) return BR_OK;
  BR_CHECK_ARG(ids && sorted_ids && sorted_pos && workspace, "brRowIndexBuild: null pointer");
  const int64_t need = brRowIndexWorkspaceBytes(n, id_type);
  if (workspace_bytes < need) {
    set_error("brRowIndexBuild: workspace %lld < required %lld", (long long)workspace_bytes, (long long)need);
    return BR_ERR_WORKSPACE;
  }
  hipStream_t s = (hipStream_t)stream;
  if (rank_path_ok(n, id_upper_bound)) {
    IdxJobs jobs;
    jobs.j[0] = jobs.j[1] = make_job(ids, sorted_ids, sorted_pos, workspace, n, id_upper_bound);
    return index_build_rank(jobs, 1, id_type, n, s);
  }
  int32_t* iota = (int32_t*)workspace;
  void* keys = (char*)workspace + align256(n * 4);
  void* tmp = (char*)keys + align256(n * 8);
  size_t tmp_bytes = (size_t)(workspace_bytes - align256(n * 4) - align256(n * 8));
  const int end_bit_cap = (id_type == BR_IDS_I64 ? 64 : 32);
  int end_bit = id_upper_bound > 0 ? bits_for(id_upper_bound + 1) : end_bit_cap;
  if (end_bit > end_bit_cap) end_bit = end_bit_cap;
  hipError_t e;
  BR_DISPATCH_ID(id_type, {
    sort_prep_kernel<IdT><<<(unsigned)ceil_div(n, 256), 256, 0, s>>>((const IdT*)ids, id_upper_bound, (IdT*)keys, iota, n);
    e = hipcub::DeviceRadixSort::SortPairs(tmp, tmp_bytes, (const IdT*)keys, (IdT*)sorted_ids, (const int32_t*)iota, sorted_pos, (int)n, 0, end_bit, s);
  });
  if (e != hipSuccess) {
    set_error("brRowIndexBuild: radix sort failed: %s", hipGetErrorString(e));
    return BR_ERR_HIP;
  }
  BR_CHECK_LAUNCH("brRowIndexBuild");
  return BR_OK;
}

extern "C" int brRowIndexBuildPair(const void* ids_a, int64_t upper_a, void* sorted_ids_a, int32_t* sorted_pos_a, void* ws_a, int64_t ws_a_bytes,
                                   const void* ids_b, int64_t upper_b, void* sorted_ids_b, int32_t* sorted_pos_b, void* ws_b, int64_t ws_b_bytes,
                                   int id_type, int64_t n, brStream stream) {
  BR_CHECK_ARG(id_type == BR_IDS_I32 || id_type == BR_IDS_I64, "brRowIndexBuildPair: bad id_type");
  if (n == 0) return BR_OK;
  if (rank_path_ok(n, upper_a) && rank_path_ok(n, upper_b)) {
    BR_CHECK_ARG(ids_a && ids_b && sorted_ids_a && sorted_ids_b && sorted_pos_a && sorted_pos_b && ws_a && ws_b, "brRowIndexBuildPair: null pointer");
    const int64_t need = brRowIndexWorkspaceBytes(n, id_type);
    if (ws_a_bytes < need || ws_b_bytes < need) {
      set_error("brRowIndexBuildPair: workspace < required %lld", (long long)need);
      return BR_ERR_WORKSPACE;
    }
    IdxJobs jobs;
    jobs.j[0] = make_job(ids_a, sorted_ids_a, sorted_pos_a, ws_a, n, upper_a);
    jobs.j[1] = make_job(ids_b, sorted_ids_b, sorted_pos_b, ws_b, n, upper_b);
    return index_build_rank(jobs, 2, id_type, n, (hipStream_t)stream);
  }
  const int rc = brRowIndexBuild(ids_a, id_type, n, upper_a, sorted_ids_a, sorted_pos_a, ws_a, ws_a_bytes, stream);
  return rc != BR_OK ? rc : brRowIndexBuild(ids_b, id_type, n, upper_b, sorted_ids_b, sorted_pos_b, ws_b, ws_b_bytes, stream);
}

extern "C" int brRowIndexBuildPairSeg(const void* ids_a, int64_t upper_a, void* sorted_ids_a, int32_t* sorted_pos_a, void* ws_a, int64_t ws_a_bytes,
                                      const void* ids_b, int64_t upper_b, void* sorted_ids_b, int32_t* sorted_pos_b, void* ws_b, int64_t ws_b_bytes,
                                      int id_type, int64_t n, int64_t seg_len, int64_t seg_stride, int64_t seg_off_a, int64_t seg_off_b, brStream stream) {
  BR_CHECK_ARG(id_type == BR_IDS_I32 || id_type == BR_IDS_I64, "brRowIndexBuildPairSeg: bad id_type");
  BR_CHECK_ARG(seg_len >= 1 && seg_stride >= seg_len && seg_off_a >= 0 && seg_off_b >= 0, "brRowIndexBuildPairSeg: bad segment geometry");
  if (n == 0) return BR_OK;
  BR_CHECK_ARG(ids_a && ids_b && sorted_ids_a && sorted_ids_b && sorted_pos_a && sorted_pos_b && ws_a && ws_b, "brRowIndexBuildPairSeg: null pointer");
  BR_CHECK_ARG(rank_path_ok(n, upper_a) && rank_path_ok(n, upper_b) && seg_phys(n - 1, seg_len, seg_stride, seg_off_a > seg_off_b ? seg_off_a : seg_off_b) < ((int64_t)1 << 31),
               "brRowIndexBuildPairSeg: n <= %lld positions and id bounds < 2^31 - 2", (long long)kRankMaxN);
  const int64_t need = brRowIndexWorkspaceBytes(n, id_type);
  if (ws_a_bytes < need || ws_b_bytes < need) { set_error("brRowIndexBuildPairSeg: workspace < required %lld", (long long)need); return BR_ERR_WORKSPACE; }
  IdxJobs jobs;
  jobs.j[0] = make_job(ids_a, sorted_ids_a, sorted_pos_a, ws_a, n, upper_a);
  jobs.j[1] = make_job(ids_b, sorted_ids_b, sorted_pos_b, ws_b, n, upper_b);
  jobs.j[0].seg_len = jobs.j[1].seg_len = seg_len; jobs.j[0].seg_stride = jobs.j[1].seg_stride = seg_stride;
  jobs.j[0].seg_off = seg_off_a; jobs.j[1].seg_off = seg_off_b;
  return index_build_rank(jobs, 2, id_type, n, (hipStream_t)stream);
}

template <typename IdT>
__global__ __launch_bounds__(256) void run_rank_kernel(IdxJobs jobs, int64_t n, int64_t run_len, int n_runs, int steps, int* err) {
  const IdxJob& job = jobs.j[blockIdx.y];
  const int64_t e = (int64_t)blockIdx.x * 256 + threadIdx.x;
  if (e >= n) return;
  const IdT* __restrict__ ids = (const IdT*)job.ids;
  auto key_at = [&](int64_t t) -> uint32_t {
    const int64_t id = (int64_t)ids[seg_phys(t, job.seg_len, job.seg_stride, job.seg_off)];
    return ((uint64_t)id < (uint64_t)job.upper) ? (uint32_t)id : job.upper;
  };
  const int r = (int)(e / run_len);
  const int64_t i = e - (int64_t)r * run_len;
  const uint32_t key = key_at(e);
  if (i > 0 && key_at(e - 1) > key && err) atomicOr(err, BR_ERRFLAG_RANGE);
  uint32_t rank = (uint32_t)i;
  constexpr int G = 8;
  for (int r0 = 0; r0 < n_runs; r0 += G) {
    uint32_t lo[G], len[G];
#pragma unroll
    for (int u = 0; u < G; ++u) {
      const int rr = r0 + u;
      const int64_t left = n - (int64_t)rr * run_len;
      len[u] = (rr < n_runs && rr != r) ? (uint32_t)(left < run_len ? left : run_len) : 0u;
      lo[u] = 0u;
    }
    for (int st = steps - 1; st >= 0; --st) {
      const uint32_t step = 1u << st;
      uint32_t v[G];
#pragma unroll
      for (int u = 0; u < G; ++u) {
        const uint32_t idx = lo[u] + step;
        const uint32_t at = idx <= len[u] ? idx - 1u : 0u;
        v[u] = key_at((int64_t)(r0 + u < n_runs ? r0 + u : 0) * run_len + at);
      }
#pragma unroll
      for (int u = 0; u < G; ++u) {
        const uint32_t idx = lo[u] + step;
        const uint32_t lt = (r0 + u < r) ? (v[u] <= key ? 1u : 0u) : (v[u] < key ? 1u : 0u);
        lo[u] += (idx <= len[u] ? lt : 0u) * step;
      }
    }
#pragma unroll
    for (int u = 0; u < G; ++u) rank += lo[u];
  }
  ((IdT*)job.sorted_ids)[rank] = (IdT)key;
  job.sorted_pos[rank] = (int32_t)seg_phys(e, job.seg_len, job.seg_stride, job.seg_off);
}

extern "C" int brRowIndexMergePairSeg(const void* ids_a, int64_t upper_a, void* sorted_ids_a, int32_t* sorted_pos_a, const void* ids_b, int64_t upper_b,
                                      void* sorted_ids_b, int32_t* sorted_pos_b, int id_type, int64_t n, int64_t seg_len, int64_t seg_stride, int64_t seg_off_a,
                                      int64_t seg_off_b, int* err_flag, brStream stream) {
  BR_CHECK_ARG(id_type == BR_IDS_I32 || id_type == BR_IDS_I64, "brRowIndexMergePairSeg: bad id_type");
  BR_CHECK_ARG(seg_len >= 1 && seg_stride >= seg_len && seg_off_a >= 0 && seg_off_b >= 0, "brRowIndexMergePairSeg: bad segment geometry");
  if (n == 0) return BR_OK;
  BR_CHECK_ARG(ids_a && ids_b && sorted_ids_a && sorted_ids_b && sorted_pos_a && sorted_pos_b, "brRowIndexMergePairSeg: null pointer");
  BR_CHECK_ARG(upper_a > 0 && upper_b > 0 && upper_a < ((int64_t)1 << 31) - 2 && upper_b < ((int64_t)1 << 31) - 2 && n < ((int64_t)1 << 31) &&
                   seg_phys(n - 1, seg_len, seg_stride, seg_off_a > seg_off_b ? seg_off_a : seg_off_b) < ((int64_t)1 << 31),
               "brRowIndexMergePairSeg: positions and id bounds < 2^31 - 2");
  IdxJobs jobs;
  jobs.j[0].ids = ids_a; jobs.j[0].sorted_ids = sorted_ids_a; jobs.j[0].sorted_pos = sorted_pos_a; jobs.j[0].upper = (uint32_t)upper_a;
  jobs.j[1].ids = ids_b; jobs.j[1].sorted_ids = sorted_ids_b; jobs.j[1].sorted_pos = sorted_pos_b; jobs.j[1].upper = (uint32_t)upper_b;
  jobs.j[0].ck = jobs.j[1].ck = nullptr; jobs.j[0].cp = jobs.j[1].cp = nullptr; jobs.j[0].end_bit = jobs.j[1].end_bit = 0;
  jobs.j[0].seg_len = jobs.j[1].seg_len = seg_len; jobs.j[0].seg_stride = jobs.j[1].seg_stride = seg_stride;
  jobs.j[0].seg_off = seg_off_a; jobs.j[1].seg_off = seg_off_b;
  const int n_runs = (int)ceil_div(n, seg_len);
  int steps = 0;
  while (((int64_t)1 << steps) <= seg_len) ++steps;
  const dim3 grid((unsigned)ceil_div(n, 256), 2);
  hipStream_t s = (hipStream_t)stream;
  BR_DISPATCH_ID(id_type, (run_rank_kernel<IdT><<<grid, 256, 0, s>>>(jobs, n, seg_len, n_runs, steps, err_flag)));
  BR_CHECK_LAUNCH("brRowIndexMergePairSeg");
  return BR_OK;
}

bool br::lookup_with_index_supported(int dim, int64_t n, int64_t upper_a, int64_t upper_b, int64_t ld_stash, const void* x0, const void* stash_a,
                                     const void* stash_b) {
  static const bool on = [] { const char* e = getenv("BR_FUSED_SORT"); return !(e && e[0] == '0'); }();
  const int wvec = wave_pair_vec(dim);
  return on && wave_rows_enabled() && wvec && ld_stash % wvec == 0 &&
         ((reinterpret_cast<uintptr_t>(x0) | reinterpret_cast<uintptr_t>(stash_a) | reinterpret_cast<uintptr_t>(stash_b)) & (4 * wvec - 1)) == 0 &&
         n > kChunkSwitchN && rank_path_ok(n, upper_a) && rank_path_ok(n, upper_b);
}
int br::lookup_with_index(const LookupArgs& la, int dim, int id_type, const IndexPairArgs& ix, brStream stream, const StepAdvance* adv) {
  const int64_t n = la.batch;
  BR_CHECK_ARG(ix.sorted_ids_a && ix.sorted_ids_b && ix.sorted_pos_a && ix.sorted_pos_b && ix.ws_a && ix.ws_b, "lookup_with_index: null pointer");
  const int64_t need = brRowIndexWorkspaceBytes(n, id_type);
  if (ix.ws_a_bytes < need || ix.ws_b_bytes < need) { set_error("lookup_with_index: workspace < required %lld", (long long)need); return BR_ERR_WORKSPACE; }
  IdxJobs jobs;
  jobs.j[0] = make_job(la.users, ix.sorted_ids_a, ix.sorted_pos_a, ix.ws_a, n, la.user_rows);
  jobs.j[1] = make_job(la.items, ix.sorted_ids_b, ix.sorted_pos_b, ix.ws_b, n, la.item_rows);
  const int n_chunks = (int)ceil_div(n, kChunkL);
  hipStream_t s = (hipStream_t)stream;
  const int wvec = wave_pair_vec(dim);
  const int ppw = wvec == 2 ? lookup_pairs_per_wave() : 1;
  const unsigned grid = (unsigned)(2 * n_chunks + ceil_div(ceil_div(n, (int64_t)(ppw < 1 ? 1 : ppw)), (int64_t)(kThreadsL / 64)));
  BR_DISPATCH_ID(id_type, {
    if (wvec == 2 && ppw == 0) lookup_sort_kernel<IdT, 2, 0><<<grid, kThreadsL, 0, s>>>(la, jobs, n, n_chunks);
    else if (wvec == 2 && ppw == 2) lookup_sort_kernel<IdT, 2, 2><<<grid, kThreadsL, 0, s>>>(la, jobs, n, n_chunks);
    else if (wvec == 2) lookup_sort_kernel<IdT, 2, 1><<<grid, kThreadsL, 0, s>>>(la, jobs, n, n_chunks);
    else lookup_sort_kernel<IdT, 4, 1><<<grid, kThreadsL, 0, s>>>(la, jobs, n, n_chunks);
  });
  BR_CHECK_LAUNCH("lookup_with_index(lookup + sort)");
  probe_split(BR_TAG_EMBED_FWD, s);
  const StepAdvance av = adv ? *adv : StepAdvance{};
  const dim3 g2((unsigned)(ceil_div(n, 256) + (av.st ? 1 : 0)), 2);
  BR_DISPATCH_ID(id_type, (chunk_rank_kernel<IdT, kChunkL><<<g2, 256, 0, s>>>(jobs, n, n_chunks, av)));
  BR_CHECK_LAUNCH("lookup_with_index(rank)");
  return BR_OK;
}

extern "C" int brGatherRowsDeferredPairWithIndex(const float* table_a, const float* m_a, const float* v_a, const int32_t* last_a, int64_t rows_a, const void* ids_a,
                                                 float* out_a, void* sorted_ids_a, int32_t* sorted_pos_a, void* ws_a, int64_t ws_a_bytes, const float* table_b,
                                                 const float* m_b, const float* v_b, const int32_t* last_b, int64_t rows_b, const void* ids_b, float* out_b,
                                                 void* sorted_ids_b, int32_t* sorted_pos_b, void* ws_b, int64_t ws_b_bytes, int dim, int id_type, int64_t n_a, int64_t n_b,
                                                 void* step_state, int advance, double lr, double beta1, double beta2, double eps, int64_t ld_out, int* err_flag,
                                                 brStream stream) {
  BR_CHECK_ARG(id_type == BR_IDS_I32 || id_type == BR_IDS_I64, "brGatherRowsDeferredPairWithIndex: bad id_type");
  BR_CHECK_ARG(table_a && m_a && v_a && last_a && ids_a && out_a && sorted_ids_a && sorted_pos_a && ws_a && table_b && m_b && v_b && last_b && ids_b && out_b &&
                   sorted_ids_b && sorted_pos_b && ws_b && step_state && rows_a > 0 && rows_b > 0 && n_a > 0 && n_b > 0 && ld_out >= dim,
               "brGatherRowsDeferredPairWithIndex: bad args");
  const int wvec = wave_row_vec(dim);
  BR_CHECK_ARG(wvec && ld_out % wvec == 0 && ((reinterpret_cast<uintptr_t>(out_a) | reinterpret_cast<uintptr_t>(out_b)) & (4 * wvec - 1)) == 0,
               "brGatherRowsDeferredPairWithIndex: rows of 64 / 128 / 256 floats (one wave per row)");
  BR_CHECK_ARG(rank_path_ok(n_a, rows_a) && rank_path_ok(n_b, rows_b), "brGatherRowsDeferredPairWithIndex: at most %lld ids per stream, table rows < 2^31 - 2", (long long)kRankMaxN);
  if (ws_a_bytes < brRowIndexWorkspaceBytes(n_a, id_type) || ws_b_bytes < brRowIndexWorkspaceBytes(n_b, id_type)) {
    set_error("brGatherRowsDeferredPairWithIndex: index workspace too small");
    return BR_ERR_WORKSPACE;
  }
  GatherDefJobs G;
  G.j[0] = GatherDefJob{table_a, m_a, v_a, last_a, rows_a, ids_a, out_a, n_a};
  G.j[1] = GatherDefJob{table_b, m_b, v_b, last_b, rows_b, ids_b, out_b, n_b};
  G.step_add = advance ? 1u : 0u;
  IdxJobs jobs;
  jobs.j[0] = make_job(ids_a, sorted_ids_a, sorted_pos_a, ws_a, n_a, rows_a);
  jobs.j[1] = make_job(ids_b, sorted_ids_b, sorted_pos_b, ws_b, n_b, rows_b);
  const int ca = (int)ceil_div(n_a, kChunkL), cb = (int)ceil_div(n_b, kChunkL);
  jobs.j[0].n = n_a; jobs.j[0].n_chunks = ca; jobs.j[1].n = n_b; jobs.j[1].n_chunks = cb;
  const AdamHp h = make_hp(0.0, beta1, beta2, eps);
  StepStateDev* ss = (StepStateDev*)step_state;
  hipStream_t s = (hipStream_t)stream;
  const int rpw = wvec == 1 ? 4 : (wvec == 2 ? 2 : 1);
  static const bool g4env = [] { const char* e = getenv("BR_GATHER_GROUP4"); return !(e && e[0] == '0'); }();
  const bool g4 = g4env && ((reinterpret_cast<uintptr_t>(table_a) | reinterpret_cast<uintptr_t>(table_b) | reinterpret_cast<uintptr_t>(m_a) | reinterpret_cast<uintptr_t>(m_b) |
                             reinterpret_cast<uintptr_t>(v_a) | reinterpret_cast<uintptr_t>(v_b) | reinterpret_cast<uintptr_t>(out_a) | reinterpret_cast<uintptr_t>(out_b)) & 15) == 0;
  const unsigned grid = (unsigned)(ca + cb + ceil_div(ceil_div(n_a + n_b, (int64_t)rpw), (int64_t)(kThreadsL / 64)));
  BR_DISPATCH_ID(id_type, BR_DISPATCH_VEC(wvec, (gather_sort_kernel<IdT, VEC><<<grid, kThreadsL, 0, s>>>(G, ss, h, ld_out, err_flag, jobs, ca, cb, g4))));
  BR_CHECK_LAUNCH("brGatherRowsDeferredPairWithIndex(gather + sort)");
  StepAdvance av;
  if (advance) { av.st = ss; av.lr = lr; av.b1 = beta1; av.b2 = beta2; }
  const int64_t nmax = n_a > n_b ? n_a : n_b;
  const dim3 g2((unsigned)(ceil_div(nmax, 256) + (advance ? 1 : 0)), 2);
  BR_DISPATCH_ID(id_type, (chunk_rank_kernel<IdT, kChunkL><<<g2, 256, 0, s>>>(jobs, nmax, ca > cb ? ca : cb, av)));
  BR_CHECK_LAUNCH("brGatherRowsDeferredPairWithIndex(rank)");
  return BR_OK;
}
```

### binary-recommendation_amd/csrc/sampling_step.hip

```cpp
#include "common.h"
#include "rows.h"
#include "adam_math.h"
#include "philox.h"
#include "sampling.h"

namespace br {

struct DrawArgs {
  const int64_t* pos_off; const void* pos_items; int64_t num_users;
  const void* cand; const uint32_t* thresh; const int32_t* alias; uint32_t n_cand;
  uint64_t seed; uint32_t step; uint32_t pos0; int max_tries;
};
struct SampleTable { const float* tab; const float* m; const float* v; const int32_t* last; int64_t rows; };
struct SampleArgs {
  DrawArgs d;
  const void* users; int64_t batch; int M;
  SampleTable user, item;
  const StepStateDev* ss; AdamHp h; int dim;
  void* out_neg; void* out_cands; float* out_scores; int* err;
};

template <typename IdT>
__device__ __forceinline__ int64_t draw_candidate(const DrawArgs& a, int64_t user, uint32_t c0, uint32_t j, int* err, const int32_t* __restrict__ last = nullptr,
                                                  int64_t rows = 0, uint32_t* seen = nullptr) {
  Positives<IdT> pos;
  pos.load(a.pos_off, (const IdT*)a.pos_items, user);
  int64_t id = 0;
  for (int t = 0; t < a.max_tries; ++t) {
    const Philox4 d = philox4x32_10(c0, j * 256u + (uint32_t)t, 5u, a.step, (uint32_t)a.seed, (uint32_t)(a.seed >> 32));
    id = candidate_of<IdT>(d, a.cand, a.thresh, a.alias, a.n_cand, err);
    if (last) *seen = (uint32_t)last[(uint64_t)id < (uint64_t)rows ? id : 0];
    if (!pos.has((IdT)id)) break;
  }
  return id;
}

template <typename IdT>
__global__ __launch_bounds__(256) void bpr_sample_one_kernel(const DrawArgs a, const IdT* __restrict__ users, int64_t batch, IdT* __restrict__ out_neg,
                                                             IdT* __restrict__ out_cands, float* __restrict__ out_scores, int* err) {
  const int64_t b = (int64_t)blockIdx.x * blockDim.x + threadIdx.x;
  if (b >= batch) return;
  int64_t u = (int64_t)users[b];
  if ((uint64_t)u >= (uint64_t)a.num_users) { if (err) atomicOr(err, BR_ERRFLAG_RANGE); u = 0; }
  const IdT id = (IdT)draw_candidate<IdT>(a, u, a.pos0 + (uint32_t)b, 0u, err);
  out_neg[b] = id;
  if (out_cands) out_cands[b] = id;
  if (out_scores) out_scores[b] = 0.f;
}

__device__ __forceinline__ float fma_chain(float acc, float4 a, float4 b) {
  return __builtin_fmaf(a.w, b.w, __builtin_fmaf(a.z, b.z, __builtin_fmaf(a.y, b.y, __builtin_fmaf(a.x, b.x, acc))));
}
__device__ __forceinline__ float fma_chain(float acc, float2 a, float2 b) { return __builtin_fmaf(a.y, b.y, __builtin_fmaf(a.x, b.x, acc)); }
__device__ __forceinline__ float fma_chain(float acc, float a, float b) { return __builtin_fmaf(a, b, acc); }

template <typename IdT, int VEC, int R, bool CHUNKED>
__global__ __launch_bounds__(256) void bpr_sample_hard_kernel(const SampleArgs a) {
  using V = typename VecT<VEC>::type;
  static_assert(!CHUNKED || VEC == 1, "chunk loop: one float per lane and pass");
  const int64_t b = (int64_t)blockIdx.x * 4 + __builtin_amdgcn_readfirstlane((int)(threadIdx.x >> 6));
  if (b >= a.batch) return;
  const int lane = (int)(threadIdx.x & 63);
  const int M = a.M, dim = a.dim;
  const StepStateDev* __restrict__ ss = a.ss;
  const bool deferred = a.user.m != nullptr;
  const uint32_t done = deferred ? ss->step : 0u;

  int64_t u = load_id((const IdT*)a.users, b);
  const bool u_csr = (uint64_t)u < (uint64_t)a.d.num_users, u_tab = (uint64_t)u < (uint64_t)a.user.rows;
  if (!(u_csr && u_tab) && a.err && lane == 0) atomicOr(a.err, BR_ERRFLAG_RANGE);
  const int64_t u_draw = u_csr ? u : 0;
  if (!u_tab) u = 0;
  const uint32_t u_seen = deferred ? (uint32_t)a.user.last[u] : done;
  const bool u_lag = u_seen < done;
  const int passes = CHUNKED ? (dim + 63) >> 6 : 1;
  V ur = vzero<VEC>(), um = vzero<VEC>(), uv = vzero<VEC>();
  if constexpr (!CHUNKED) {
    const int64_t uo = u * dim + lane * VEC;
    ur = vload<VEC>(a.user.tab + uo);
    if (u_lag) { um = vload<VEC>(a.user.m + uo); uv = vload<VEC>(a.user.v + uo); }
  }
  int64_t mine = 0, drawn = 0;
  uint32_t mine_seen = done;
  if (lane < M) {
    mine = draw_candidate<IdT>(a.d, u_draw, a.d.pos0 + (uint32_t)b, (uint32_t)lane, a.err, deferred ? a.item.last : nullptr, a.item.rows, &mine_seen);
    drawn = mine;
    if (a.out_cands) ((IdT*)a.out_cands)[b * M + lane] = (IdT)mine;
    if ((uint64_t)mine >= (uint64_t)a.item.rows) { if (a.err) atomicOr(a.err, BR_ERRFLAG_RANGE); mine = -1; }
  }
  const int id_lo = (int)(uint32_t)mine, id_hi = (int)(uint32_t)((uint64_t)mine >> 32), id_seen = (int)mine_seen;

  float best = -__builtin_inff();
  int best_j = 0;
  for (int g = 0; g < M; g += R) {
    int64_t row[R];
    uint32_t seen[R];
#pragma unroll
    for (int q = 0; q < R; ++q) {
      const int j = g + q < M ? g + q : M - 1;
      row[q] = (int64_t)(((uint64_t)(uint32_t)__builtin_amdgcn_readlane(id_hi, j) << 32) | (uint64_t)(uint32_t)__builtin_amdgcn_readlane(id_lo, j));
      if (row[q] < 0) row[q] = 0;
      seen[q] = (uint32_t)__builtin_amdgcn_readlane(id_seen, j);
    }
    float acc[R];
#pragma unroll
    for (int q = 0; q < R; ++q) acc[q] = 0.f;
    for (int p = 0; p < passes; ++p) {
      const int col = CHUNKED ? p * 64 + lane : lane * VEC;
      const bool in = !CHUNKED || col < dim;
      if constexpr (CHUNKED) {
        const int64_t uo = u * dim + col;
        ur = in ? vload<VEC>(a.user.tab + uo) : vzero<VEC>();
        um = vzero<VEC>(); uv = vzero<VEC>();
        if (u_lag && in) { um = vload<VEC>(a.user.m + uo); uv = vload<VEC>(a.user.v + uo); }
      }
      V th[R], m[R], v[R];
#pragma unroll
      for (int q = 0; q < R; ++q) {
        const int64_t off = row[q] * dim + col;
        th[q] = in ? vload<VEC>(a.item.tab + off) : vzero<VEC>();
        m[q] = vzero<VEC>(); v[q] = vzero<VEC>();
        if (seen[q] < done && in) { m[q] = vload<VEC>(a.item.m + off); v[q] = vload<VEC>(a.item.v + off); }
      }
      if (u_lag && (CHUNKED || g == 0)) adam_catch_up_uniform<false>(ur, um, uv, u_seen, done, ss, a.h);
#pragma unroll
      for (int q = 0; q < R; ++q) {
        if (seen[q] < done) adam_catch_up_uniform<false>(th[q], m[q], v[q], seen[q], done, ss, a.h);
        acc[q] = fma_chain(acc[q], ur, th[q]);
      }
    }
#pragma unroll
    for (int q = 0; q < R; ++q) {
      float s = acc[q];
      s += __shfl_xor(s, 32, 64);
      s += __shfl_xor(s, 16, 64);
      s += __shfl_xor(s, 8, 64);
      s += __shfl_xor(s, 4, 64);
      s += __shfl_xor(s, 2, 64);
      s += __shfl_xor(s, 1, 64);
      const float sc = __builtin_bit_cast(float, __builtin_amdgcn_readfirstlane(__builtin_bit_cast(int, s)));
      const int j = g + q;
      if (j < M) {
        if (a.out_scores && lane == 0) a.out_scores[b * M + j] = sc;
        if (sc > best) { best = sc; best_j = j; }
      }
    }
  }
  if (lane == best_j) ((IdT*)a.out_neg)[b] = (IdT)drawn;
}

}

using namespace br;

extern "C" int brBprSampleNegatives(const void* users, int id_type, int64_t batch, int64_t pos0, uint32_t draw_step, const int64_t* pos_off,
                                    const void* pos_items, int64_t num_users, const void* cand_items, int64_t n_cand, const uint32_t* alias_thresh,
                                    const int32_t* alias_slot, uint64_t seed, int n_candidates, int max_tries, const float* user_table,
                                    const float* user_m, const float* user_v, const int32_t* user_last, int64_t user_rows, const float* item_table,
                                    const float* item_m, const float* item_v, const int32_t* item_last, int64_t item_rows, int dim,
                                    const void* step_state, double beta1, double beta2, double eps, void* out_neg, void* out_cands,
                                    float* out_scores, int* err_flag, brStream stream) {
  BR_CHECK_ARG(id_type == BR_IDS_I32 || id_type == BR_IDS_I64, "brBprSampleNegatives: bad id_type");
  BR_CHECK_ARG(n_candidates >= 1 && n_candidates <= 32, "brBprSampleNegatives: n_candidates %d out of [1, 32]", n_candidates);
  BR_CHECK_ARG(max_tries >= 1 && max_tries <= 256, "brBprSampleNegatives: max_tries %d out of [1, 256]", max_tries);
  BR_CHECK_ARG(batch >= 0 && batch < ((int64_t)1 << 31) && pos0 >= 0 && num_users >= 1 && n_cand >= 1 && n_cand < ((int64_t)1 << 32),
               "brBprSampleNegatives: bad sizes");
  BR_CHECK_ARG((alias_thresh == nullptr) == (alias_slot == nullptr), "brBprSampleNegatives: alias_thresh and alias_slot: both or neither");
  const bool hard = n_candidates > 1;
  if (hard) {
    BR_CHECK_ARG(user_table && item_table && user_rows > 0 && item_rows > 0 && dim >= 1, "brBprSampleNegatives: n_candidates > 1 scores the candidates: tables required");
    const bool any = user_m || user_v || user_last || item_m || item_v || item_last;
    const bool all = user_m && user_v && user_last && item_m && item_v && item_last && step_state;
    BR_CHECK_ARG(!any || all, "brBprSampleNegatives: deferred tables need m, v, last of both tables and the step state; current tables none of them");
  }
  if (batch == 0) return BR_OK;
  BR_CHECK_ARG(users && pos_off && pos_items && out_neg, "brBprSampleNegatives: null pointer");
  const DrawArgs d{pos_off, pos_items, num_users, cand_items, alias_thresh, alias_slot, (uint32_t)n_cand, seed, draw_step, (uint32_t)pos0, max_tries};
  hipStream_t s = (hipStream_t)stream;
  if (!hard) {
    BR_DISPATCH_ID(id_type, (bpr_sample_one_kernel<IdT><<<(unsigned)ceil_div(batch, 256), 256, 0, s>>>(d, (const IdT*)users, batch, (IdT*)out_neg, (IdT*)out_cands, out_scores, err_flag)));
    BR_CHECK_LAUNCH("brBprSampleNegatives");
    return BR_OK;
  }
  SampleArgs a{};
  a.d = d; a.users = users; a.batch = batch; a.M = n_candidates;
  a.user = SampleTable{user_table, user_m, user_v, user_last, user_rows};
  a.item = SampleTable{item_table, item_m, item_v, item_last, item_rows};
  a.ss = (const StepStateDev*)step_state; a.h = make_hp(0.0, beta1, beta2, eps); a.dim = dim;
  a.out_neg = out_neg; a.out_cands = out_cands; a.out_scores = out_scores; a.err = err_flag;
  const unsigned grid = (unsigned)ceil_div(batch, 4);
  constexpr int R = 4;
  const int wvec = wave_row_vec(dim);
  const uintptr_t al = reinterpret_cast<uintptr_t>(user_table) | reinterpret_cast<uintptr_t>(item_table) | reinterpret_cast<uintptr_t>(user_m) |
                       reinterpret_cast<uintptr_t>(user_v) | reinterpret_cast<uintptr_t>(item_m) | reinterpret_cast<uintptr_t>(item_v);
  if (wvec && (al & (4 * wvec - 1)) == 0) {
    BR_DISPATCH_ID(id_type, BR_DISPATCH_VEC(wvec, (bpr_sample_hard_kernel<IdT, VEC, R, false><<<grid, 256, 0, s>>>(a))));
  } else {
    BR_DISPATCH_ID(id_type, (bpr_sample_hard_kernel<IdT, 1, R, true><<<grid, 256, 0, s>>>(a)));
  }
  BR_CHECK_LAUNCH("brBprSampleNegatives");
  return BR_OK;
}
```

Before: 216.5 million pairs/s.

## Load step-state scalars via constant address space and prefetch alpha history for replay

Reads the step state and alpha history through address-space-4 (constant/scalar) pointers, batched into a ReplayK struct pinned to SGPRs. The first eight alpha values for each row's replay are prefetched one row ahead, and the next eight are software-pipelined inside the fast replay loop. Error flags become a single atomicOr after the work instead of per-row stores. The intent is to turn per-row scalar-memory latency in lookup and gather kernels into overlapped scalar loads, at the cost of more SGPR pressure and some speculative prefetches. The sampling kernel is moved onto the old per-call path.

```diff
diff --git a/binary-recommendation_amd/csrc/adam_math.h b/binary-recommendation_amd/csrc/adam_math.h
--- a/binary-recommendation_amd/csrc/adam_math.h
+++ b/binary-recommendation_amd/csrc/adam_math.h
@@ -76,9 +76,160 @@
   for (uint32_t j = from + 1; j <= upto; ++j) adam_decay(th, m, v, ring[j & (BR_ALPHA_RING - 1)], h);
 }
 
-template <typename V>
-__device__ __forceinline__ void adam_replay_uniform(V& th, V& m, V& v, uint32_t from, uint32_t upto, const StepStateDev* __restrict__ ss,
-                                                    const AdamHp& h) {
+typedef const StepStateDev __attribute__((address_space(4)))* StepStateK;
+__device__ __forceinline__ StepStateK step_state_k(const StepStateDev* ss) { return (StepStateK)ss; }
+
+struct ReplayK {
+  uint32_t step, fast, trunc;
+  float sqrt_b2, eps_c;
+};
+__device__ __forceinline__ ReplayK replay_k(const StepStateDev* ss) {
+  const StepStateK k = step_state_k(ss);
+  return ReplayK{k->step, k->fast, k->trunc, k->sqrt_b2, k->eps_c};
+}
+#if defined(__HIP_DEVICE_COMPILE__)
+#define BR_PIN_K(k) asm volatile("" : "+s"((k).step), "+s"((k).fast), "+s"((k).trunc), "+s"((k).sqrt_b2), "+s"((k).eps_c))
+#define BR_PIN_K1(k, x) asm volatile("" : "+s"((k).step), "+s"((k).fast), "+s"((k).trunc), "+s"((k).sqrt_b2), "+s"((k).eps_c), "+s"(x))
+#define BR_PIN_K2(k, x, y) asm volatile("" : "+s"((k).step), "+s"((k).fast), "+s"((k).trunc), "+s"((k).sqrt_b2), "+s"((k).eps_c), "+s"(x), "+s"(y))
+#else
+#define BR_PIN_K(k) (void)(k)
+#define BR_PIN_K1(k, x) (void)(k), (void)(x)
+#define BR_PIN_K2(k, x, y) (void)(k), (void)(x), (void)(y)
+#endif
+__device__ __forceinline__ void replay_k_pin(ReplayK& k) { BR_PIN_K(k); }
+struct Alpha8 { float a[8]; };
+__device__ __forceinline__ Alpha8 alpha8(const StepStateDev* ss, uint32_t j) {
+  const float __attribute__((address_space(4)))* rp = step_state_k(ss)->alpha_hist + (j & (BR_ALPHA_RING - 1));
+  Alpha8 r;
+#pragma unroll
+  for (int q = 0; q < 8; ++q) r.a[q] = rp[q];
+  return r;
+}
+
+template <typename V>
+__device__ __forceinline__ void adam_replay_uniform(V& th, V& m, V& v, uint32_t from, uint32_t upto, const StepStateDev* ss, const AdamHp& h) {
+  if (__builtin_amdgcn_ballot_w64(!(all_zero(m) && all_zero(v))) == 0) return;
+  const StepStateK k = step_state_k(ss);
+  float a = k->alpha_hist[(from + 1) & (BR_ALPHA_RING - 1)];
+  for (uint32_t j = from + 1; j <= upto; ++j) {
+    const float an = k->alpha_hist[(j + 1) & (BR_ALPHA_RING - 1)];
+    adam_decay(th, m, v, a, h);
+    a = an;
+  }
+}
+
+struct FastRp {
+  float c, eps_c;
+  uint32_t trunc;
+};
+__device__ __forceinline__ FastRp fast_rp(const StepStateDev* __restrict__ ss) { return FastRp{ss->sqrt_b2, ss->eps_c, ss->trunc}; }
+__device__ __forceinline__ FastRp fast_rp(const ReplayK& k) { return FastRp{k.sqrt_b2, k.eps_c, k.trunc}; }
+
+__device__ __forceinline__ void fast_open(pk2 v, float eps, pk2& d, pk2& r) {
+  d = (pk2){__builtin_amdgcn_sqrtf(v.x), __builtin_amdgcn_sqrtf(v.y)} + eps;
+  r = (pk2){__builtin_amdgcn_rcpf(d.x), __builtin_amdgcn_rcpf(d.y)};
+}
+__device__ __forceinline__ void fast_open(float v, float eps, float& d, float& r) {
+  d = __builtin_amdgcn_sqrtf(v) + eps;
+  r = __builtin_amdgcn_rcpf(d);
+}
+__device__ __forceinline__ void fast_step(pk2& th, pk2& m, pk2& d, pk2& r, float alpha, float b1, const FastRp& f) {
+  m = m * b1;
+  d = __builtin_elementwise_fma(d, (pk2){f.c, f.c}, (pk2){f.eps_c, f.eps_c});
+  r = r * __builtin_elementwise_fma(-d, r, (pk2){2.f, 2.f});
+  th = __builtin_elementwise_fma(-(m * alpha), r, th);
+}
+__device__ __forceinline__ void fast_step(float& th, float& m, float& d, float& r, float alpha, float b1, const FastRp& f) {
+  m = m * b1;
+  d = __builtin_fmaf(d, f.c, f.eps_c);
+  r = r * __builtin_fmaf(-d, r, 2.f);
+  th = __builtin_fmaf(-(m * alpha), r, th);
+}
+template <typename V> struct FastSt;
+template <> struct FastSt<float> {
+  float th, m, d, r;
+  __device__ __forceinline__ void open(float t, float mm, float v, float eps) { th = t; m = mm; fast_open(v, eps, d, r); }
+  __device__ __forceinline__ void step(float a, float b1, const FastRp& f) { fast_step(th, m, d, r, a, b1, f); }
+  __device__ __forceinline__ float theta() const { return th; }
+};
+template <> struct FastSt<float2> {
+  pk2 th, m, d, r;
+  __device__ __forceinline__ void open(float2 t, float2 mm, float2 v, float eps) { th = (pk2){t.x, t.y}; m = (pk2){mm.x, mm.y}; fast_open((pk2){v.x, v.y}, eps, d, r); }
+  __device__ __forceinline__ void step(float a, float b1, const FastRp& f) { fast_step(th, m, d, r, a, b1, f); }
+  __device__ __forceinline__ float2 theta() const { return make_float2(th.x, th.y); }
+};
+template <> struct FastSt<float4> {
+  pk2 th0, m0, d0, r0, th1, m1, d1, r1;
+  __device__ __forceinline__ void open(float4 t, float4 mm, float4 v, float eps) {
+    th0 = (pk2){t.x, t.y}; m0 = (pk2){mm.x, mm.y}; fast_open((pk2){v.x, v.y}, eps, d0, r0);
+    th1 = (pk2){t.z, t.w}; m1 = (pk2){mm.z, mm.w}; fast_open((pk2){v.z, v.w}, eps, d1, r1);
+  }
+  __device__ __forceinline__ void step(float a, float b1, const FastRp& f) { fast_step(th0, m0, d0, r0, a, b1, f); fast_step(th1, m1, d1, r1, a, b1, f); }
+  __device__ __forceinline__ float4 theta() const { return make_float4(th0.x, th0.y, th1.x, th1.y); }
+};
+__device__ __forceinline__ uint32_t pow_index(uint32_t k) { return k < (uint32_t)BR_ALPHA_RING ? k : (uint32_t)BR_ALPHA_RING - 1u; }
+
+template <typename V>
+__device__ __forceinline__ void fast_moments(V& m, V& v, uint32_t lag, const StepStateDev* __restrict__ ss) {
+  const uint32_t k = pow_index(lag);
+  m = vmul(m, ss->pow1[k]);
+  v = vmul(v, ss->pow2[k]);
+}
+
+__device__ __forceinline__ uint32_t fast_end(uint32_t from, uint32_t upto, const ReplayK& k) {
+  const uint32_t lag = upto - from;
+  return from + (lag < k.trunc ? lag : k.trunc);
+}
+__device__ __forceinline__ Alpha8 fast_first(const StepStateDev* ss, uint32_t from) { return alpha8(ss, from + 1); }
+template <typename V>
+__device__ __forceinline__ void adam_replay_fast_uniform(V& th, const V& m, const V& v, uint32_t from, uint32_t upto, const ReplayK& k, const Alpha8& first,
+                                                         const StepStateDev* ss, const AdamHp& h) {
+  if (__builtin_amdgcn_ballot_w64(!(all_zero(m) && all_zero(v))) == 0) return;
+  const FastRp f = fast_rp(k);
+  const uint32_t end = fast_end(from, upto, k);
+  FastSt<V> st;
+  st.open(th, m, v, h.eps);
+  uint32_t j = from + 1;
+  Alpha8 cur = first;
+  for (; j + 7 <= end; j += 8) {
+    const Alpha8 nxt = alpha8(ss, j + 8);
+#pragma unroll
+    for (int q = 0; q < 8; ++q) st.step(cur.a[q], h.b1, f);
+    cur = nxt;
+  }
+  const uint32_t rem = end + 1 - j;
+#pragma unroll
+  for (int q = 0; q < 7; ++q) {
+    if ((uint32_t)q >= rem) break;
+    st.step(cur.a[q], h.b1, f);
+  }
+  th = st.theta();
+}
+template <typename V>
+__device__ __forceinline__ void adam_replay_fast(V& th, const V& m, const V& v, uint32_t from, uint32_t upto, const float* ring, const FastRp& f,
+                                                 const AdamHp& h) {
+  if (all_zero(m) && all_zero(v)) return;
+  const uint32_t lag = upto - from;
+  const uint32_t end = from + (lag < f.trunc ? lag : f.trunc);
+  FastSt<V> st;
+  st.open(th, m, v, h.eps);
+  for (uint32_t j = from + 1; j <= end; ++j) st.step(ring[j & (BR_ALPHA_RING - 1)], h.b1, f);
+  th = st.theta();
+}
+
+template <bool MOMENTS, typename V>
+__device__ __forceinline__ void adam_catch_up_uniform(V& th, V& m, V& v, uint32_t from, uint32_t upto, const ReplayK& k, const Alpha8& first,
+                                                      const StepStateDev* ss, const AdamHp& h) {
+  if (k.fast) {
+    adam_replay_fast_uniform(th, m, v, from, upto, k, first, ss, h);
+    if (MOMENTS) fast_moments(m, v, upto - from, ss);
+  } else {
+    adam_replay_uniform(th, m, v, from, upto, ss, h);
+  }
+}
+template <typename V>
+__device__ __forceinline__ void adam_replay_uniform_percall(V& th, V& m, V& v, uint32_t from, uint32_t upto, const StepStateDev* __restrict__ ss,
+                                                            const AdamHp& h) {
   if (__builtin_amdgcn_ballot_w64(!(all_zero(m) && all_zero(v))) == 0) return;
   float a = ss->alpha_hist[(from + 1) & (BR_ALPHA_RING - 1)];
   for (uint32_t j = from + 1; j <= upto; ++j) {
@@ -87,67 +238,9 @@
     a = an;
   }
 }
-
-struct FastRp {
-  float c, eps_c;
-  uint32_t trunc;
-};
-__device__ __forceinline__ FastRp fast_rp(const StepStateDev* __restrict__ ss) { return FastRp{ss->sqrt_b2, ss->eps_c, ss->trunc}; }
-
-__device__ __forceinline__ void fast_open(pk2 v, float eps, pk2& d, pk2& r) {
-  d = (pk2){__builtin_amdgcn_sqrtf(v.x), __builtin_amdgcn_sqrtf(v.y)} + eps;
-  r = (pk2){__builtin_amdgcn_rcpf(d.x), __builtin_amdgcn_rcpf(d.y)};
-}
-__device__ __forceinline__ void fast_open(float v, float eps, float& d, float& r) {
-  d = __builtin_amdgcn_sqrtf(v) + eps;
-  r = __builtin_amdgcn_rcpf(d);
-}
-__device__ __forceinline__ void fast_step(pk2& th, pk2& m, pk2& d, pk2& r, float alpha, float b1, const FastRp& f) {
-  m = m * b1;
-  d = __builtin_elementwise_fma(d, (pk2){f.c, f.c}, (pk2){f.eps_c, f.eps_c});
-  r = r * __builtin_elementwise_fma(-d, r, (pk2){2.f, 2.f});
-  th = __builtin_elementwise_fma(-(m * alpha), r, th);
-}
-__device__ __forceinline__ void fast_step(float& th, float& m, float& d, float& r, float alpha, float b1, const FastRp& f) {
-  m = m * b1;
-  d = __builtin_fmaf(d, f.c, f.eps_c);
-  r = r * __builtin_fmaf(-d, r, 2.f);
-  th = __builtin_fmaf(-(m * alpha), r, th);
-}
-template <typename V> struct FastSt;
-template <> struct FastSt<float> {
-  float th, m, d, r;
-  __device__ __forceinline__ void open(float t, float mm, float v, float eps) { th = t; m = mm; fast_open(v, eps, d, r); }
-  __device__ __forceinline__ void step(float a, float b1, const FastRp& f) { fast_step(th, m, d, r, a, b1, f); }
-  __device__ __forceinline__ float theta() const { return th; }
-};
-template <> struct FastSt<float2> {
-  pk2 th, m, d, r;
-  __device__ __forceinline__ void open(float2 t, float2 mm, float2 v, float eps) { th = (pk2){t.x, t.y}; m = (pk2){mm.x, mm.y}; fast_open((pk2){v.x, v.y}, eps, d, r); }
-  __device__ __forceinline__ void step(float a, float b1, const FastRp& f) { fast_step(th, m, d, r, a, b1, f); }
-  __device__ __forceinline__ float2 theta() const { return make_float2(th.x, th.y); }
-};
-template <> struct FastSt<float4> {
-  pk2 th0, m0, d0, r0, th1, m1, d1, r1;
-  __device__ __forceinline__ void open(float4 t, float4 mm, float4 v, float eps) {
-    th0 = (pk2){t.x, t.y}; m0 = (pk2){mm.x, mm.y}; fast_open((pk2){v.x, v.y}, eps, d0, r0);
-    th1 = (pk2){t.z, t.w}; m1 = (pk2){mm.z, mm.w}; fast_open((pk2){v.z, v.w}, eps, d1, r1);
-  }
-  __device__ __forceinline__ void step(float a, float b1, const FastRp& f) { fast_step(th0, m0, d0, r0, a, b1, f); fast_step(th1, m1, d1, r1, a, b1, f); }
-  __device__ __forceinline__ float4 theta() const { return make_float4(th0.x, th0.y, th1.x, th1.y); }
-};
-__device__ __forceinline__ uint32_t pow_index(uint32_t k) { return k < (uint32_t)BR_ALPHA_RING ? k : (uint32_t)BR_ALPHA_RING - 1u; }
-
-template <typename V>
-__device__ __forceinline__ void fast_moments(V& m, V& v, uint32_t lag, const StepStateDev* __restrict__ ss) {
-  const uint32_t k = pow_index(lag);
-  m = vmul(m, ss->pow1[k]);
-  v = vmul(v, ss->pow2[k]);
-}
-
-template <typename V>
-__device__ __forceinline__ void adam_replay_fast_uniform(V& th, const V& m, const V& v, uint32_t from, uint32_t upto, const StepStateDev* __restrict__ ss,
-                                                         const AdamHp& h) {
+template <typename V>
+__device__ __forceinline__ void adam_replay_fast_uniform_percall(V& th, const V& m, const V& v, uint32_t from, uint32_t upto,
+                                                                 const StepStateDev* __restrict__ ss, const AdamHp& h) {
   if (__builtin_amdgcn_ballot_w64(!(all_zero(m) && all_zero(v))) == 0) return;
   const FastRp f = fast_rp(ss);
   const uint32_t lag = upto - from;
@@ -166,25 +259,14 @@
   for (; j <= end; ++j) st.step(ss->alpha_hist[j & (BR_ALPHA_RING - 1)], h.b1, f);
   th = st.theta();
 }
-template <typename V>
-__device__ __forceinline__ void adam_replay_fast(V& th, const V& m, const V& v, uint32_t from, uint32_t upto, const float* ring, const FastRp& f,
-                                                 const AdamHp& h) {
-  if (all_zero(m) && all_zero(v)) return;
-  const uint32_t lag = upto - from;
-  const uint32_t end = from + (lag < f.trunc ? lag : f.trunc);
-  FastSt<V> st;
-  st.open(th, m, v, h.eps);
-  for (uint32_t j = from + 1; j <= end; ++j) st.step(ring[j & (BR_ALPHA_RING - 1)], h.b1, f);
-  th = st.theta();
-}
-
 template <bool MOMENTS, typename V>
-__device__ __forceinline__ void adam_catch_up_uniform(V& th, V& m, V& v, uint32_t from, uint32_t upto, const StepStateDev* __restrict__ ss, const AdamHp& h) {
+__device__ __forceinline__ void adam_catch_up_uniform_percall(V& th, V& m, V& v, uint32_t from, uint32_t upto, const StepStateDev* __restrict__ ss,
+                                                              const AdamHp& h) {
   if (ss->fast) {
-    adam_replay_fast_uniform(th, m, v, from, upto, ss, h);
+    adam_replay_fast_uniform_percall(th, m, v, from, upto, ss, h);
     if (MOMENTS) fast_moments(m, v, upto - from, ss);
   } else {
-    adam_replay_uniform(th, m, v, from, upto, ss, h);
+    adam_replay_uniform_percall(th, m, v, from, upto, ss, h);
   }
 }
 template <bool MOMENTS, typename V>
diff --git a/binary-recommendation_amd/csrc/gather.hip b/binary-recommendation_amd/csrc/gather.hip
--- a/binary-recommendation_amd/csrc/gather.hip
+++ b/binary-recommendation_amd/csrc/gather.hip
@@ -234,16 +234,20 @@
   const int64_t b = (int64_t)blockIdx.x * 4 + __builtin_amdgcn_readfirstlane((int)(threadIdx.x >> 6));
   if (b >= n) return;
   const int lane = (int)(threadIdx.x & 63);
+  ReplayK k = replay_k(ss);
   int64_t r = load_id(ids, b);
+  BR_PIN_K1(k, r);
   const bool ok = (uint64_t)r < (uint64_t)rows;
-  if (!ok) { if (err && lane == 0) *err = 1; r = 0; }
-  const uint32_t t = ss->step, seen = (uint32_t)last[r];
+  if (!ok) r = 0;
+  const uint32_t t = k.step, seen = (uint32_t)last[r];
   const int64_t off = r * dim + lane * VEC;
   V th = vload<VEC>(table + off);
   if (seen + 1 < t) {
     V m = vload<VEC>(M + off), v = vload<VEC>(Vv + off);
-    adam_catch_up_uniform<false>(th, m, v, seen, t - 1, ss, h);
-  }
+    const Alpha8 first = fast_first(ss, seen);
+    adam_catch_up_uniform<false>(th, m, v, seen, t - 1, k, first, ss, h);
+  }
+  flag_range(err, ok, lane == 0);
   vstore<VEC>(out + b * ld_out + lane * VEC, ok ? th : vzero<VEC>());
 }
 
diff --git a/binary-recommendation_amd/csrc/lookup_wave.h b/binary-recommendation_amd/csrc/lookup_wave.h
--- a/binary-recommendation_amd/csrc/lookup_wave.h
+++ b/binary-recommendation_amd/csrc/lookup_wave.h
@@ -22,28 +22,44 @@
   return (uint32_t)forced & 3u;
 }
 
+template <typename IdT>
+__device__ __forceinline__ ReplayK load_k_id_pair(const StepStateDev* ss, const IdT* users, const IdT* items, int64_t b, int64_t& u, int64_t& i) {
+  typedef const IdT __attribute__((address_space(4)))* IdK;
+  ReplayK k = replay_k(ss);
+  IdT uu = *(users ? (IdK)users + b : (IdK)ss), ii = *(items ? (IdK)items + b : (IdK)ss);
+  BR_PIN_K2(k, uu, ii);
+  u = users ? (int64_t)uu : b;
+  i = items ? (int64_t)ii : b;
+  return k;
+}
+__device__ __forceinline__ void flag_range(int* err, bool ok, bool writer) {
+  if (!ok && err && writer) atomicOr(err, BR_ERRFLAG_RANGE);
+}
+
 template <typename IdT, int VEC>
 __device__ __forceinline__ void lookup_wave_pair(const LookupArgs& a, int64_t b, int lane) {
   using V = typename VecT<VEC>::type;
   constexpr int dim = 32 * VEC;
   constexpr int64_t ld = 2 * dim;
   const float* __restrict__ user_tab = a.user_tab; const float* __restrict__ item_tab = a.item_tab;
-  const StepStateDev* __restrict__ ss = a.ss;
+  const StepStateDev* ss = a.ss;
   const int col = lane * VEC;
-  int64_t u = load_id((const IdT*)a.users, b), i = load_id((const IdT*)a.items, b);
+  int64_t u, i;
+  const ReplayK k = load_k_id_pair(ss, (const IdT*)a.users, (const IdT*)a.items, b, u, i);
   const bool uok = (uint64_t)u < (uint64_t)a.user_rows, iok = (uint64_t)i < (uint64_t)a.item_rows;
-  if ((!uok || !iok) && a.err && lane == 0) *a.err = 1;
   if (!uok) u = 0;
   if (!iok) i = 0;
-  const uint32_t t = ss->step + a.step_add;
+  const uint32_t t = k.step + a.step_add;
   const uint32_t lu = (uint32_t)a.user_last[u], li = (uint32_t)a.item_last[i];
   const int64_t uo = u * ld + col, io = i * ld + col;
   V ur = vload<VEC>(user_tab + uo), ir = vload<VEC>(item_tab + io);
   V um = vzero<VEC>(), uv = vzero<VEC>(), im = vzero<VEC>(), iv = vzero<VEC>();
   if ((a.spec & 1u) || lu + 1 < t) { um = vload<VEC>(a.user_m + uo); uv = vload<VEC>(a.user_v + uo); }
   if ((a.spec & 2u) || li + 1 < t) { im = vload<VEC>(a.item_m + io); iv = vload<VEC>(a.item_v + io); }
-  if (li + 1 < t) adam_catch_up_uniform<false>(ir, im, iv, li, t - 1, ss, a.h);
-  if (lu + 1 < t) adam_catch_up_uniform<false>(ur, um, uv, lu, t - 1, ss, a.h);
+  const Alpha8 ia = fast_first(ss, li), ua = fast_first(ss, lu);
+  if (li + 1 < t) adam_catch_up_uniform<false>(ir, im, iv, li, t - 1, k, ia, ss, a.h);
+  if (lu + 1 < t) adam_catch_up_uniform<false>(ur, um, uv, lu, t - 1, k, ua, ss, a.h);
+  flag_range(a.err, uok && iok, lane == 0);
   if (!uok) ur = vzero<VEC>();
   if (!iok) ir = vzero<VEC>();
   const bool mlp = lane < 32;
@@ -72,22 +88,23 @@
 __device__ __forceinline__ void lookup_half_pair(const LookupArgs& a, int64_t b, int lane) {
   constexpr int dim = 64;
   constexpr int64_t ld = 2 * dim;
-  const StepStateDev* __restrict__ ss = a.ss;
+  const StepStateDev* ss = a.ss;
   const bool it = lane >= 32;
   const int col = (lane & 31) * 4;
-  int64_t u = load_id((const IdT*)a.users, b), i = load_id((const IdT*)a.items, b);
+  int64_t u, i;
+  const ReplayK rk = load_k_id_pair(ss, (const IdT*)a.users, (const IdT*)a.items, b, u, i);
   const bool uok = (uint64_t)u < (uint64_t)a.user_rows, iok = (uint64_t)i < (uint64_t)a.item_rows;
-  if ((!uok || !iok) && a.err && lane == 0) *a.err = 1;
   if (!uok) u = 0;
   if (!iok) i = 0;
-  const uint32_t t = ss->step + a.step_add;
+  const uint32_t t = rk.step + a.step_add;
   const uint32_t lu = (uint32_t)a.user_last[u], li = (uint32_t)a.item_last[i];
-  const FastRp f = fast_rp(ss);
+  const FastRp f = fast_rp(rk);
   uint32_t lag_u = lu + 1 < t ? t - 1 - lu : 0u, lag_i = li + 1 < t ? t - 1 - li : 0u;
   const int64_t off = (it ? i : u) * ld + col;
   const float4 th = vload<4>((it ? a.item_tab : a.user_tab) + off);
   float4 m = vzero<4>(), v = vzero<4>();
   if (it ? lag_i > 0 : lag_u > 0) { m = vload<4>((it ? a.item_m : a.user_m) + off); v = vload<4>((it ? a.item_v : a.user_v) + off); }
+  Alpha8 au = fast_first(ss, lu), ai = fast_first(ss, li);
   float4 out = th;
   lag_u = lag_u < f.trunc ? lag_u : f.trunc; lag_i = lag_i < f.trunc ? lag_i : f.trunc;
   const uint32_t steps = lag_u > lag_i ? lag_u : lag_i, mine = it ? lag_i : lag_u;
@@ -96,20 +113,19 @@
     st.open(th, m, v, a.h.eps);
     uint32_t k = 1;
     for (; k + 7 <= steps; k += 8) {
-      const float* __restrict__ ru = ss->alpha_hist + ((lu + k) & (BR_ALPHA_RING - 1));
-      const float* __restrict__ ri = ss->alpha_hist + ((li + k) & (BR_ALPHA_RING - 1));
-      float au[8], ai[8];
-#pragma unroll
-      for (int q = 0; q < 8; ++q) { au[q] = ru[q]; ai[q] = ri[q]; }
-#pragma unroll
-      for (int q = 0; q < 8; ++q) st.step(k + q <= mine ? (it ? ai[q] : au[q]) : 0.f, a.h.b1, f);
-    }
-    for (; k <= steps; ++k) {
-      const float au = ss->alpha_hist[(lu + k) & (BR_ALPHA_RING - 1)], ai = ss->alpha_hist[(li + k) & (BR_ALPHA_RING - 1)];
-      st.step(k <= mine ? (it ? ai : au) : 0.f, a.h.b1, f);
+      const Alpha8 nu = alpha8(ss, lu + k + 8), ni = alpha8(ss, li + k + 8);
+#pragma unroll
+      for (int q = 0; q < 8; ++q) st.step(k + q <= mine ? (it ? ai.a[q] : au.a[q]) : 0.f, a.h.b1, f);
+      au = nu; ai = ni;
+    }
+#pragma unroll
+    for (int q = 0; q < 7; ++q) {
+      if (k + q > steps) break;
+      st.step(k + q <= mine ? (it ? ai.a[q] : au.a[q]) : 0.f, a.h.b1, f);
     }
     out = st.theta();
   }
+  flag_range(a.err, uok && iok, lane == 0);
   if (it ? !iok : !uok) out = vzero<4>();
   const bool mlp = col < dim;
   const int uoff = a.item_first ? dim : 0, ioff = a.item_first ? 0 : dim;
@@ -131,22 +147,33 @@
   constexpr int dim = 32 * VEC;
   constexpr int64_t ld = 2 * dim;
   const float* __restrict__ user_tab = a.user_tab; const float* __restrict__ item_tab = a.item_tab;
-  const StepStateDev* __restrict__ ss = a.ss;
+  const StepStateDev* ss = a.ss;
   const int col = lane * VEC;
-  const uint32_t t = ss->step + a.step_add;
+  ReplayK k = replay_k(ss);
   int64_t u[R], i[R], bq[R];
   bool live[R], uok[R], iok[R];
 #pragma unroll
   for (int q = 0; q < R; ++q) {
     live[q] = b0 + q < a.batch;
     bq[q] = live[q] ? b0 + q : a.batch - 1;
-    u[q] = load_id((const IdT*)a.users, bq[q]); i[q] = load_id((const IdT*)a.items, bq[q]);
-  }
+  }
+  {
+    typedef const IdT __attribute__((address_space(4)))* IdK;
+    IdT uu[R], ii[R];
+#pragma unroll
+    for (int q = 0; q < R; ++q) { uu[q] = *(a.users ? (IdK)a.users + bq[q] : (IdK)ss); ii[q] = *(a.items ? (IdK)a.items + bq[q] : (IdK)ss); }
+#pragma unroll
+    for (int q = 0; q < R; ++q) { BR_PIN_K2(k, uu[q], ii[q]); }
+#pragma unroll
+    for (int q = 0; q < R; ++q) { u[q] = a.users ? (int64_t)uu[q] : bq[q]; i[q] = a.items ? (int64_t)ii[q] : bq[q]; }
+  }
+  const uint32_t t = k.step + a.step_add;
   uint32_t lu[R], li[R];
+  bool all_ok = true;
 #pragma unroll
   for (int q = 0; q < R; ++q) {
     uok[q] = (uint64_t)u[q] < (uint64_t)a.user_rows; iok[q] = (uint64_t)i[q] < (uint64_t)a.item_rows;
-    if ((!uok[q] || !iok[q]) && a.err && lane == 0 && live[q]) *a.err = 1;
+    all_ok = all_ok && ((uok[q] && iok[q]) || !live[q]);
     if (!uok[q]) u[q] = 0;
     if (!iok[q]) i[q] = 0;
     lu[q] = (uint32_t)a.user_last[u[q]]; li[q] = (uint32_t)a.item_last[i[q]];
@@ -162,10 +189,13 @@
   }
   const bool mlp = lane < 32;
   const int uoff = a.item_first ? dim : 0, ioff = a.item_first ? 0 : dim;
-#pragma unroll
-  for (int q = 0; q < R; ++q) {
-    if (li[q] + 1 < t) adam_catch_up_uniform<false>(ir[q], im[q], iv[q], li[q], t - 1, ss, a.h);
-    if (lu[q] + 1 < t) adam_catch_up_uniform<false>(ur[q], um[q], uv[q], lu[q], t - 1, ss, a.h);
+  Alpha8 ia = fast_first(ss, li[0]), ua = fast_first(ss, lu[0]);
+#pragma unroll
+  for (int q = 0; q < R; ++q) {
+    const Alpha8 ic = ia, uc = ua;
+    if (q + 1 < R) { ia = fast_first(ss, li[q + 1]); ua = fast_first(ss, lu[q + 1]); }
+    if (li[q] + 1 < t) adam_catch_up_uniform<false>(ir[q], im[q], iv[q], li[q], t - 1, k, ic, ss, a.h);
+    if (lu[q] + 1 < t) adam_catch_up_uniform<false>(ur[q], um[q], uv[q], lu[q], t - 1, k, uc, ss, a.h);
     if (!uok[q]) ur[q] = vzero<VEC>();
     if (!iok[q]) ir[q] = vzero<VEC>();
     if (!live[q]) continue;
@@ -189,6 +219,7 @@
     if constexpr (VEC == 4) s += __shfl_xor(s, 1, 64);
     if (lane == 63) a.dot[b] = s;
   }
+  flag_range(a.err, all_ok, lane == 0);
 }
 
 struct GatherDefJob { const float* table; const float* M; const float* Vv; const int32_t* last; int64_t rows; const void* ids; float* out; int64_t n; int64_t seg_off = 0; };
@@ -198,31 +229,35 @@
   uint32_t step_add = 0;
 };
 template <typename IdT, int VEC>
-__device__ __forceinline__ void gather_deferred_wave_row(const GatherDefJobs& jobs, const GatherDefJob& jb, int64_t b, int lane, const StepStateDev* __restrict__ ss,
+__device__ __forceinline__ void gather_deferred_wave_row(const GatherDefJobs& jobs, const GatherDefJob& jb, int64_t b, int lane, const StepStateDev* ss,
                                                          const AdamHp& h, int64_t ld_out, int* err) {
   using V = typename VecT<VEC>::type;
   constexpr int dim = 64 * VEC;
   b = seg_phys(b, jobs.seg_len, jobs.seg_stride, jb.seg_off);
+  ReplayK k = replay_k(ss);
   int64_t r = load_id((const IdT*)jb.ids, b);
+  BR_PIN_K1(k, r);
   const bool ok = (uint64_t)r < (uint64_t)jb.rows;
-  if (!ok) { if (err && lane == 0) *err = 1; r = 0; }
-  const uint32_t t = ss->step + jobs.step_add, seen = (uint32_t)jb.last[r];
+  if (!ok) r = 0;
+  const uint32_t t = k.step + jobs.step_add, seen = (uint32_t)jb.last[r];
   const int64_t off = r * dim + lane * VEC;
   V th = vload<VEC>(jb.table + off);
   if (seen + 1 < t) {
     V m = vload<VEC>(jb.M + off), v = vload<VEC>(jb.Vv + off);
-    adam_catch_up_uniform<false>(th, m, v, seen, t - 1, ss, h);
-  }
+    const Alpha8 first = fast_first(ss, seen);
+    adam_catch_up_uniform<false>(th, m, v, seen, t - 1, k, first, ss, h);
+  }
+  flag_range(err, ok, lane == 0);
   vstore<VEC>(jb.out + b * ld_out + lane * VEC, ok ? th : vzero<VEC>());
 }
 
 template <typename IdT, int VEC, int R>
-__device__ __forceinline__ void gather_deferred_wave_rows(const GatherDefJobs& jobs, int64_t b0, int lane, const StepStateDev* __restrict__ ss, const AdamHp& h,
+__device__ __forceinline__ void gather_deferred_wave_rows(const GatherDefJobs& jobs, int64_t b0, int lane, const StepStateDev* ss, const AdamHp& h,
                                                           int64_t ld_out, int* err) {
   using V = typename VecT<VEC>::type;
   constexpr int dim = 64 * VEC;
   const int64_t n_a = jobs.j[0].n, n_all = n_a + jobs.j[1].n;
-  const uint32_t t = ss->step + jobs.step_add;
+  ReplayK k = replay_k(ss);
   int which[R];
   int64_t pos[R], row[R];
   bool live[R], ok[R];
@@ -236,12 +271,16 @@
     pos[q] = seg_phys(which[q] ? bc - n_a : bc, jobs.seg_len, jobs.seg_stride, jb.seg_off);
     row[q] = load_id((const IdT*)jb.ids, pos[q]);
   }
+  replay_k_pin(k);
+  const uint32_t t = k.step + jobs.step_add;
   uint32_t seen[R];
+  bool all_ok = true;
 #pragma unroll
   for (int q = 0; q < R; ++q) {
     const GatherDefJob& jb = jobs.j[which[q]];
     ok[q] = (uint64_t)row[q] < (uint64_t)jb.rows;
-    if (!ok[q]) { if (err && lane == 0 && live[q]) *err = 1; row[q] = 0; }
+    all_ok = all_ok && (ok[q] || !live[q]);
+    if (!ok[q]) row[q] = 0;
     seen[q] = (uint32_t)jb.last[row[q]];
   }
   V th[R], m[R], v[R];
@@ -253,11 +292,15 @@
     m[q] = vzero<VEC>(); v[q] = vzero<VEC>();
     if (seen[q] + 1 < t) { m[q] = vload<VEC>(jb.M + off); v[q] = vload<VEC>(jb.Vv + off); }
   }
-#pragma unroll
-  for (int q = 0; q < R; ++q) {
-    if (seen[q] + 1 < t) adam_catch_up_uniform<false>(th[q], m[q], v[q], seen[q], t - 1, ss, h);
+  Alpha8 first = fast_first(ss, seen[0]);
+#pragma unroll
+  for (int q = 0; q < R; ++q) {
+    const Alpha8 cur = first;
+    if (q + 1 < R) first = fast_first(ss, seen[q + 1]);
+    if (seen[q] + 1 < t) adam_catch_up_uniform<false>(th[q], m[q], v[q], seen[q], t - 1, k, cur, ss, h);
     if (live[q]) vstore<VEC>(jobs.j[which[q]].out + pos[q] * ld_out + lane * VEC, ok[q] ? th[q] : vzero<VEC>());
   }
+  flag_range(err, all_ok, lane == 0);
 }
 
 template <typename IdT>
@@ -277,7 +320,7 @@
   int64_t row = which ? load_id((const IdT*)jb.ids, pos) : load_id((const IdT*)ja.ids, pos);
   const int64_t rows = which ? jb.rows : ja.rows;
   const bool ok = (uint64_t)row < (uint64_t)rows;
-  if (!ok) { if (err && live && (lane & 15) == 0) *err = 1; row = 0; }
+  if (!ok) { if (err && live && (lane & 15) == 0) atomicOr(err, BR_ERRFLAG_RANGE); row = 0; }
   const uint32_t seen = (uint32_t)(which ? jb.last : ja.last)[row];
   const FastRp f = fast_rp(ss);
   uint32_t lag = seen + 1 < t ? t - 1 - seen : 0u;
diff --git a/binary-recommendation_amd/csrc/row_index.hip b/binary-recommendation_amd/csrc/row_index.hip
--- a/binary-recommendation_amd/csrc/row_index.hip
+++ b/binary-recommendation_amd/csrc/row_index.hip
@@ -355,7 +355,8 @@
 
 bool br::lookup_with_index_supported(int dim, int64_t n, int64_t upper_a, int64_t upper_b, int64_t ld_stash, const void* x0, const void* stash_a,
                                      const void* stash_b) {
-  static const bool on = [] { const char* e = getenv("BR_FUSED_SORT"); return !(e && e[0] == '0'); }();
+  const char* e = getenv("BR_FUSED_SORT");
+  const bool on = !(e && e[0] == '0');
   const int wvec = wave_pair_vec(dim);
   return on && wave_rows_enabled() && wvec && ld_stash % wvec == 0 &&
          ((reinterpret_cast<uintptr_t>(x0) | reinterpret_cast<uintptr_t>(stash_a) | reinterpret_cast<uintptr_t>(stash_b)) & (4 * wvec - 1)) == 0 &&
diff --git a/binary-recommendation_amd/csrc/sampling_step.hip b/binary-recommendation_amd/csrc/sampling_step.hip
--- a/binary-recommendation_amd/csrc/sampling_step.hip
+++ b/binary-recommendation_amd/csrc/sampling_step.hip
@@ -122,10 +122,10 @@
         m[q] = vzero<VEC>(); v[q] = vzero<VEC>();
         if (seen[q] < done && in) { m[q] = vload<VEC>(a.item.m + off); v[q] = vload<VEC>(a.item.v + off); }
       }
-      if (u_lag && (CHUNKED || g == 0)) adam_catch_up_uniform<false>(ur, um, uv, u_seen, done, ss, a.h);
+      if (u_lag && (CHUNKED || g == 0)) adam_catch_up_uniform_percall<false>(ur, um, uv, u_seen, done, ss, a.h);
 #pragma unroll
       for (int q = 0; q < R; ++q) {
-        if (seen[q] < done) adam_catch_up_uniform<false>(th[q], m[q], v[q], seen[q], done, ss, a.h);
+        if (seen[q] < done) adam_catch_up_uniform_percall<false>(th[q], m[q], v[q], seen[q], done, ss, a.h);
         acc[q] = fma_chain(acc[q], ur, th[q]);
       }
     }
```

Measured after the change: 224.3 million pairs/s (median of 6 runs). 1.04x the previous value.
